# sleep3r/Diffusion-Handwriting-Generation.pytorch

Hardware: AMD Instinct MI355X
Metric: stroke-points/sec reverse-sampled (T=60, L=488) (higher is better)
Workload: dtype bf16; 1 GPU; configs[1]: batch=64 prompts/GPU, T=60, L=488, Lt=30, d_model=128/192/256, num_layers=2, diffusion_mode=new, random-init weights; global_batch=64, seq_len=488, parallelism=batch-shard x1 (no collectives)

## Files before the change

### diffusion-handwriting-generation.pytorch_amd/csrc/convblock.hip

```cpp
#include <algorithm>
#include <cstdlib>
#include "convblock_core.h"

namespace {

template <typename T, int BM, int CO, int NW, int OCC = 1, int UPC = 0, int CH = 0, int CIN = 0, int TIGHT = 0, int PP = 0>
__global__ __launch_bounds__(NW * 64) __attribute__((amdgpu_waves_per_eu(OCC * NW / 4, (OCC * NW / 4) < 2 ? 2 : OCC * NW / 4)))
void convblock_kernel(const ConvBlockParams p, const EncChain nx) {
  extern __shared__ __attribute__((aligned(16))) char smem[];
  constexpr int BMO = TIGHT == 2 ? BM : BM - 2 - 2 * TIGHT;
  const int tiles = (p.L + BMO - 1) / BMO;
  const int bid = xcd_swizzle(blockIdx.x, gridDim.x);
  convblock_body<T, BM, CO, NW, OCC, UPC, CH, CIN, TIGHT, PP>(p, nx, bid / tiles, (bid % tiles) * BMO, smem);
}

template <typename T, int BM, int CO, int NW, int OCC = 1, int UPC = 0, int CH = 0, int CIN = 0, int TIGHT = 0, int PP = 0>
hipError_t launch_t(const ConvBlockParams& p, hipStream_t st, const EncChain* nx = nullptr) {
  size_t lds = lds_bytes<T, BM, CO>(p.Cin, UPC ? p.up_cin : 0, TIGHT == 2 ? BM + 16 : BM);
  if (CH) lds = std::max(lds, (size_t)2 * BM * tile_stride<T>(CO) + 2 * 8 * BM * sizeof(float) + enc_a_text_kv_bytes<T, CO, BM>() + enc_a_param_bytes<T, CO>());
  if (lds > 160 * 1024 || (UPC && (p.Cin != UPC || p.up_cin % 32)) || (CH != 0) != (nx != nullptr)) return hipErrorInvalidValue;
  if (CIN && (p.Cin != CIN || (UPC && p.up_cin != up_skip_width<UPC>()))) return hipErrorInvalidValue;
  constexpr int BMO = TIGHT == 2 ? BM : BM - 2 - 2 * TIGHT;
  const int tiles = (p.L + BMO - 1) / BMO;
  hipLaunchKernelGGL((convblock_kernel<T, BM, CO, NW, OCC, UPC, CH, CIN, TIGHT, PP>), dim3(p.B * tiles), dim3(NW * 64), lds, st, p, nx ? *nx : EncChain{});
  return hipGetLastError();
}

template <typename T, int BM, int CO, int NW, int OCC = 1, int UPC = 0, int CH = 0, int CIN = 0, int TIGHT = 0, int PP = 0>
hipError_t attr() {
  return hipFuncSetAttribute(reinterpret_cast<const void*>(convblock_kernel<T, BM, CO, NW, OCC, UPC, CH, CIN, TIGHT, PP>),
                             hipFuncAttributeMaxDynamicSharedMemorySize, 160 * 1024);
}

constexpr int enc_cin(int CO) { return CO == 256 ? 192 : 128; }

}

hipError_t convblock_init() {
  hipError_t e;
#define A(...) if ((e = attr<__VA_ARGS__>()) != hipSuccess) return e
  A(bf16_t, 64, 128, 8); A(bf16_t, 128, 128, 8); A(bf16_t, 64, 128, 8, 2, 0, 0, 128); A(bf16_t, 64, 192, 8, 2, 0, 0, 128); A(bf16_t, 64, 192, 8);
  A(bf16_t, 64, 256, 8); A(bf16_t, 32, 256, 8); A(bf16_t, 48, 256, 8);
  A(bf16_t, 64, 128, 8, 1, 0, 0, 128); A(bf16_t, 128, 128, 8, 1, 0, 0, 128); A(bf16_t, 64, 192, 8, 1, 0, 0, 128);
  A(bf16_t, 64, 256, 8, 1, 0, 0, 192); A(bf16_t, 48, 256, 8, 1, 0, 0, 192);
  A(bf16_t, 64, 128, 8, 1, 192, 0, 192); A(bf16_t, 128, 128, 8, 1, 192, 0, 192); A(bf16_t, 64, 192, 8, 1, 256, 0, 256);
  A(bf16_t, 64, 256, 8, 1, 384, 0, 384); A(bf16_t, 48, 256, 8, 1, 384, 0, 384);
  A(bf16_t, 128, 128, 8, 1, 192, 0, 192, 1); A(bf16_t, 48, 256, 8, 1, 384, 0, 384, 1);
  A(bf16_t, 128, 128, 8, 1, 0, 0, 128, 0, 1); A(bf16_t, 128, 128, 8, 1, 192, 0, 192, 1, 1); A(bf16_t, 128, 128, 8, 1, 192, 0, 192, 0, 1);
  A(bf16_t, 32, 256, 8, 1, 0, 0, 192, 2); A(bf16_t, 32, 256, 8, 1, 384, 0, 384, 2);
  A(bf16_t, 64, 192, 8, 1, 0, 1, 128); A(bf16_t, 48, 256, 8, 1, 0, 1, 192); A(bf16_t, 64, 256, 8, 1, 0, 1, 192);
  A(bf16_t, 32, 256, 8, 1, 0, 1, 192, 2);
  A(float, 32, 128, 4); A(float, 32, 192, 4); A(float, 32, 256, 4);
#undef A
  return hipSuccess;
}

static long conv_wgs() {
  const char* e = getenv("DHW_CONV_WGS");
  return e ? atol(e) : 256;
}

static bool use_bm48(const ConvBlockParams& p) {
  if (const char* e = getenv("DHW_CONV_BM")) return atoi(e) == 48;
  const long t64 = (long)p.B * ((p.L + 61) / 62), t48 = (long)p.B * ((p.L + 45) / 46);
  return t64 < conv_wgs() && t48 <= conv_wgs() && t48 > t64;
}

static bool use_asym32(const ConvBlockParams& p) {
  static const bool on = !(getenv("DHW_CONV_ASYM") && atoi(getenv("DHW_CONV_ASYM")) == 0);
  if (!on || getenv("DHW_CONV_BM")) return false;
  const long t32 = (long)p.B * ((p.L + 31) / 32), t46 = (long)p.B * ((p.L + 45) / 46);
  return t32 <= conv_wgs() && t32 > t46;
}

static int conv_pp() {
  const char* e = getenv("DHW_CONV_PP");
  return e ? atoi(e) : 0;
}

hipError_t launch_convblock(int prec, const ConvBlockParams& p_in, hipStream_t st) {
  ConvBlockParams p = p_in;
  if (const char* e = getenv("DHW_CONV_STAGGER")) p.stagger = atoi(e);
  if (p.Cin % 32 || (p.L & 1) || (p.pool && p.out_f32) || (p.fuse_heads && !p.out_f32) || (!p.out && !p.fuse_heads)) return hipErrorInvalidValue;
  static const bool rt = getenv("DHW_CONV_RT") && atoi(getenv("DHW_CONV_RT"));
  if (p.up_h) {
    if (prec != PREC_BF16 || p.strokes || !p.up_w || !p.up_b || !p.up_low) return hipErrorInvalidValue;
    static const bool tight_ok = !(getenv("DHW_CONV_TIGHT") && atoi(getenv("DHW_CONV_TIGHT")) == 0);
    auto tight = [&](int bm) { return tight_ok && (p.L + bm - 5) / (bm - 4) == (p.L + bm - 3) / (bm - 2); };
    if (p.Cout == 128 && p.Cin == 192 && p.up_cin == 128) {
      const bool big = (long)p.B * ((p.L + 61) / 62) > conv_wgs() && lds_bytes<bf16_t, 128, 128>(p.Cin, p.up_cin) <= 160 * 1024;
      if (big && (conv_pp() & 2)) return tight(128) ? launch_t<bf16_t, 128, 128, 8, 1, 192, 0, 192, 1, 1>(p, st) : launch_t<bf16_t, 128, 128, 8, 1, 192, 0, 192, 0, 1>(p, st);
      if (big && tight(128)) return launch_t<bf16_t, 128, 128, 8, 1, 192, 0, 192, 1>(p, st);
      return big ? launch_t<bf16_t, 128, 128, 8, 1, 192, 0, 192>(p, st) : launch_t<bf16_t, 64, 128, 8, 1, 192, 0, 192>(p, st);
    }
    if (p.Cout == 192 && p.Cin == 256 && p.up_cin == 192) return launch_t<bf16_t, 64, 192, 8, 1, 256, 0, 256>(p, st);
    if (p.Cout == 256 && p.Cin == 384 && p.up_cin == 256) {
      if (use_asym32(p)) return launch_t<bf16_t, 32, 256, 8, 1, 384, 0, 384, 2>(p, st);
      if (use_bm48(p) && tight(48)) return launch_t<bf16_t, 48, 256, 8, 1, 384, 0, 384, 1>(p, st);
      return use_bm48(p) ? launch_t<bf16_t, 48, 256, 8, 1, 384, 0, 384>(p, st) : launch_t<bf16_t, 64, 256, 8, 1, 384, 0, 384>(p, st);
    }
    return hipErrorInvalidValue;
  }
  if (prec == PREC_BF16) {
    const bool sk = !rt && p.Cin == enc_cin(p.Cout);
    switch (p.Cout) {
      case 128: {
        const bool big = (long)p.B * ((p.L + 61) / 62) > conv_wgs() && lds_bytes<bf16_t, 128, 128>(p.Cin) <= 160 * 1024 &&
                         !(getenv("DHW_CONV_BM") && atoi(getenv("DHW_CONV_BM")) == 64);
        if (getenv("DHW_CONV_OCC") && atoi(getenv("DHW_CONV_OCC")) == 2 && sk && lds_bytes<bf16_t, 64, 128>(p.Cin) <= 80 * 1024)
          return launch_t<bf16_t, 64, 128, 8, 2, 0, 0, 128>(p, st);
        if (sk && big && (conv_pp() & 1)) return launch_t<bf16_t, 128, 128, 8, 1, 0, 0, 128, 0, 1>(p, st);
        if (sk) return big ? launch_t<bf16_t, 128, 128, 8, 1, 0, 0, 128>(p, st) : launch_t<bf16_t, 64, 128, 8, 1, 0, 0, 128>(p, st);
        return big ? launch_t<bf16_t, 128, 128, 8>(p, st) : launch_t<bf16_t, 64, 128, 8>(p, st);
      }
      case 192:
        if (getenv("DHW_CONV_OCC") && atoi(getenv("DHW_CONV_OCC")) == 2 && sk && lds_bytes<bf16_t, 64, 192>(p.Cin) <= 80 * 1024)
          return launch_t<bf16_t, 64, 192, 8, 2, 0, 0, 128>(p, st);
        return sk ? launch_t<bf16_t, 64, 192, 8, 1, 0, 0, 128>(p, st) : launch_t<bf16_t, 64, 192, 8>(p, st);
      case 256:
        if (sk && use_asym32(p)) return launch_t<bf16_t, 32, 256, 8, 1, 0, 0, 192, 2>(p, st);
        if (use_bm48(p)) return sk ? launch_t<bf16_t, 48, 256, 8, 1, 0, 0, 192>(p, st) : launch_t<bf16_t, 48, 256, 8>(p, st);
        if (getenv("DHW_CONV_BM") && atoi(getenv("DHW_CONV_BM")) == 32) return launch_t<bf16_t, 32, 256, 8>(p, st);
        return sk ? launch_t<bf16_t, 64, 256, 8, 1, 0, 0, 192>(p, st) : launch_t<bf16_t, 64, 256, 8>(p, st);
    }
  } else {
    switch (p.Cout) {
      case 128: return launch_t<float, 32, 128, 4>(p, st);
      case 192: return launch_t<float, 32, 192, 4>(p, st);
      case 256: return launch_t<float, 32, 256, 4>(p, st);
    }
  }
  return hipErrorInvalidValue;
}

bool convblock_chain_supported(int prec, const ConvBlockParams& p, const EncChain& chain) {
  if (prec != PREC_BF16 || chain.mode != 1 || chain.a.x || p.up_h || p.strokes || p.out_f32 || p.fuse_heads) return false;
  if (chain.a.d != p.Cout || chain.a.Lk != p.L || chain.a.B != p.B || (p.L & 1)) return false;
  if (getenv("DHW_CONV_BM") || getenv("DHW_CONV_OCC")) return false;
  return (p.Cout == 192 || p.Cout == 256) && p.Cin == enc_cin(p.Cout) && enclayer_supported(prec, chain.a.d, chain.a.heads);
}

bool convblock_chain_auto(const ConvBlockParams& p) { return p.Cout == 256 && use_asym32(p); }

hipError_t launch_convblock_chain(int prec, const ConvBlockParams& p, const EncChain& chain, hipStream_t st) {
  if (!convblock_chain_supported(prec, p, chain) || p.Cin % 32 || (!p.out)) return hipErrorInvalidValue;
  if (p.Cout == 192) return launch_t<bf16_t, 64, 192, 8, 1, 0, 1, 128>(p, st, &chain);
  if (use_asym32(p)) return launch_t<bf16_t, 32, 256, 8, 1, 0, 1, 192, 2>(p, st, &chain);
  return use_bm48(p) ? launch_t<bf16_t, 48, 256, 8, 1, 0, 1, 192>(p, st, &chain) : launch_t<bf16_t, 64, 256, 8, 1, 0, 1, 192>(p, st, &chain);
}
```

### diffusion-handwriting-generation.pytorch_amd/csrc/convblock_core.h

```cpp
#pragma once
#include <algorithm>
#include "enc_a_core.h"
#include "heads_core.h"

namespace {

#define CB_SILU(x) ((DHW_ABL & 8) ? (x) : silu_t<T>(x))
#define CB_SILU_TILES(NT_, MT_, v) do { if constexpr (!(DHW_ABL & 8)) silu_tiles2<T, NT_, MT_>(v); } while (0)
#define CB_BARRIER() do { if constexpr (!(DHW_ABL & 64)) lds_barrier(); } while (0)

#define STAMP(slot) DHW_STAMP_IF(p.stamps && (int)blockIdx.x == p.stagger && (threadIdx.x & 63) == 0, (threadIdx.x >> 6) * 16 + slot, __builtin_amdgcn_s_memrealtime())

template <typename T, int BM> __host__ __device__ constexpr int h2_stride(int CO) { return BM >= 128 ? CO * (int)sizeof(T) + 16 : tile_stride<T>(CO); }

template <int NT>
struct Epi {
  f32x4 bias[NT], gam[NT], bet[NT];
  DHW_DEV void load(const float* b, const float* g, const float* be, int n0) {
#pragma unroll
    for (int i = 0; i < NT; ++i) {
      bias[i] = *reinterpret_cast<const f32x4*>(b + n0 + 16 * i);
      gam[i] = *reinterpret_cast<const f32x4*>(g + n0 + 16 * i);
      bet[i] = *reinterpret_cast<const f32x4*>(be + n0 + 16 * i);
    }
  }
  DHW_DEV void load_bias(const float* b, int n0) {
#pragma unroll
    for (int i = 0; i < NT; ++i) {
      bias[i] = *reinterpret_cast<const f32x4*>(b + n0 + 16 * i);
      gam[i] = (f32x4){1, 1, 1, 1};
      bet[i] = (f32x4){0, 0, 0, 0};
    }
  }
};

template <int UPC> constexpr int up_skip_width() { return UPC == 384 ? 256 : UPC == 256 ? 192 : UPC == 192 ? 128 : 0; }
template <typename T, int BM, int CO, int NW, int OCC = 1, int UPC = 0, int CH = 0, int CIN = 0, int TIGHT = 0, int PP = 0, typename P, typename X>
DHW_DEV void convblock_body(const P& p, const X& nx, const int b, const int m0, char* smem) {
  constexpr int ES = sizeof(T), NTHR = NW * 64;
  constexpr bool SK = CIN != 0;
  constexpr int KT1 = 3 * CIN / 32;
  static_assert(UPC == 0 || CIN == 0 || CIN == UPC, "a fused input stage produces the block's own input width");
  constexpr bool ASYM = TIGHT == 2;
  constexpr int BMO = ASYM ? BM : BM - 2 - 2 * TIGHT;
  constexpr int RX = BMO + 4;
  constexpr int BM1 = ASYM ? BM + 16 : BM;
  constexpr int C1 = CO / 2;
  constexpr int T1 = C1 / 16, T2 = CO / 16;
  constexpr int WN1 = NW == 8 ? (T1 >= 8 ? 8 : (T1 == 6 ? 6 : 4)) : 2;
  constexpr int WM1 = NW == 8 ? (T1 >= 6 ? 1 : 2) : 2;
  constexpr bool TALL = NW == 8 && BM >= 128 && T2 == 8;
  constexpr int WN2 = NW == 8 ? (TALL ? 4 : (T2 % 8 == 0 ? 8 : 6)) : 4;
  constexpr int WM2 = TALL ? 2 : 1;
  constexpr int MT1 = BM1 / WM1 / 16, NT1 = T1 / WN1;
  constexpr int MT2 = BM / WM2 / 16, NT2 = T2 / WN2;
  static_assert(NT1 * WN1 == T1 && NT2 * WN2 == T2 && MT1 * 16 * WM1 == BM1 && WM1 * WN1 <= NW && WM2 * WN2 <= NW, "unsupported tile / wave layout");
  static_assert(!ASYM || WM1 == 1, "the asymmetric tiling: blocks with one row group in conv1");
  constexpr bool PPX = PP != 0;
  static_assert(!PPX || (TALL && WM1 == 2 && WN1 == 4 && CH == 0 && !ASYM && OCC == 1), "ping-pong: the 2 x 4 wave layouts of the tall tiles");
  constexpr int RING = (ES == 2 ? 24 : 12) * (CO == 256 ? 2 : 3) / 3 / (OCC * NW > 8 ? OCC : 1);

  const int Ls = sample_len(p.lens, p.lsh, b, p.L);
  if constexpr (DHW_LENS) { if (m0 >= Ls) return; }
  const int tid = body_tid(), lane = tid & 63, wave = __builtin_amdgcn_readfirstlane(tid >> 6);
  const int l15 = lane & 15, g = lane >> 4;
  const int Cin = SK ? CIN : p.Cin;
  const bool pp_lead = PPX && __builtin_amdgcn_readfirstlane(wave) >= NW / 2;
#define PP_BARRIER() do { if constexpr (PPX) CB_BARRIER(); } while (0)

  const int SX = tile_stride<T>(Cin), SH1 = tile_stride<T>(C1), SH2 = h2_stride<T, BM>(CO);
  char* XS = smem;
  char* XR = XS + RX * SX;
  char* H1 = XR + RX * SX;
  char* H2 = H1 + (BM1 + 2) * SH1;
  const float* gam = p.film + (size_t)b * p.film_bs;
  const float* bet = gam + p.film_tot;

  const bool act1 = WM1 * WN1 == NW || wave < WM1 * WN1, act2 = WM2 * WN2 == NW || wave < WM2 * WN2;
  const int wm1 = act1 ? wave / WN1 : 0, wn1 = act1 ? wave % WN1 : 0, row01 = wm1 * (BM1 / WM1), nt01 = wn1 * NT1;
  const int wm2 = act2 ? wave / WN2 : 0, wn2 = act2 ? wave % WN2 : 0, row02 = wm2 * (BM / WM2), nt02 = wn2 * NT2;
  const int n1 = nt01 * 16 + 4 * g, n2 = nt02 * 16 + 4 * g;
  const int KCin = Cin / 32;

  if constexpr (OCC == 2) {
    if (p.stagger && blockIdx.x >= gridDim.x / 2)
      for (int i = 0; i < p.stagger; ++i) __builtin_amdgcn_s_sleep(16);
  }
  STAMP(0);
  WRing<T, NT1, RING> ring1;
  Epi<NT1> ep1;
  auto fill1 = [&]() {
    const T* w = reinterpret_cast<const T*>(p.w_c1) + ((size_t)nt01 * KCin * 3 * 64 + lane) * 8;
    if constexpr (SK) ring1.template fill_s<KT1>(w);
    else ring1.fill(w, KCin * 3);
  };

  if constexpr (UPC != 0) {
    constexpr int RXP = (RX + 15) / 16 * 16, RH = RXP + 2, MTU = RXP / 16;
    constexpr int TU = UPC / 16, WNU = TU % 8 == 0 ? 8 : 4, WMU = NW / WNU, NTU = TU / WNU;
    constexpr int MTG = (MTU + WMU - 1) / WMU;
    static_assert(NTU * WNU == TU && NW == 8, "unsupported input width");
    const int wmu = wave / WNU, wnu = wave % WNU;
    const int ntu0 = wnu * NTU, nu = ntu0 * 16 + 4 * g, rowu0 = wmu * MTG * 16;
    constexpr int UCH = up_skip_width<UPC>();
    const int Ch = SK ? UCH : p.up_cin, KCh = Ch / 32, SHh = tile_stride<T>(Ch);
    char* HS = H1;
    WRing<T, NTU, (NTU * MTG >= 24 ? 12 : RING)> ringu;
    Epi<NTU> epu;
    {
      constexpr int CPRH = UCH * ES / 16, CPX = UPC * ES / 16;
      constexpr int UH = (RH * CPRH + NTHR - 1) / NTHR, UL = (RX * CPX + NTHR - 1) / NTHR;
      static_assert(SK, "the fused input stage is compiled for static widths");
      const char* src = reinterpret_cast<const char*>(p.up_h);
      const char* low = reinterpret_cast<const char*>(p.up_low);
      CopyRegs<UH> ch;
      CopyRegs<UL> cl;
      ch.load(RH * CPRH, tid, NTHR, [&](int id) { const int r = id / CPRH, cc = id - r * CPRH, lrow = min(max(m0 - 3 + r, 0), p.L - 1);
                                                  return reinterpret_cast<const uint4*>(src + ((size_t)(b * p.L + lrow) * UCH) * ES + (size_t)cc * 16); });
      cl.load(RX * CPX, tid, NTHR, [&](int id) { const int r = id / CPX, cc = id - r * CPX, lrow = min(max(m0 - 2 + r, 0), p.L - 1);
                                                 return reinterpret_cast<const uint4*>(low + ((size_t)(b * (p.L / 2) + (lrow >> 1)) * UPC) * ES + (size_t)cc * 16); });
      ch.store(RH * CPRH, tid, NTHR, [&](int id) { const int r = id / CPRH, cc = id - r * CPRH; return reinterpret_cast<uint4*>(HS + r * SHh + cc * 16); },
               [&](int id) { const int lrow = m0 - 3 + id / CPRH; return lrow >= 0 && lrow < Ls; });
      cl.store(RX * CPX, tid, NTHR, [&](int id) { const int r = id / CPX, cc = id - r * CPX; return reinterpret_cast<uint4*>(XR + r * SX + cc * 16); },
               [&](int id) { const int lrow = m0 - 2 + id / CPX; return lrow >= 0 && lrow < Ls; });
    }
    ringu.template fill_s<3 * UCH / 32>(reinterpret_cast<const T*>(p.up_w) + ((size_t)ntu0 * KCh * 3 * 64 + lane) * 8);
    epu.load_bias(p.up_b, nu);
    CB_BARRIER();
    STAMP(10);
    f32x4 acc[NTU][MTG];
    acc_zero(acc);
    ringu.template run_s<MTG, 3 * UCH / 32>(acc, HS + (rowu0 + l15) * SHh + g * 8 * ES, SHh, KCh);
    STAMP(11);
    if (act1) {
      fill1();
      ep1.load(p.b_c1, gam + p.f1, bet + p.f1, n1);
    }
    {
      auto keep = [&](int j) { const int lrow = m0 - 2 + rowu0 + j * 16 + l15; return lrow >= 0 && lrow < Ls; };
      auto valid = [&](int j) { return rowu0 + j * 16 + l15 < RX; };
#pragma unroll
      for (int i = 0; i < NTU; ++i)
#pragma unroll
        for (int j = 0; j < MTG; ++j) {
          const int r = min(rowu0 + j * 16 + l15, RX - 1);
          acc[i][j] = round_to<T>(acc[i][j] + epu.bias[i] + load4(reinterpret_cast<const T*>(XR + r * SX) + nu + 16 * i));
        }
      store_tiles<T, NTU, MTG>(lane, XR, SX, rowu0, nu, acc, keep, valid);
      CB_SILU_TILES(NTU, MTG, acc);
      store_tiles<T, NTU, MTG>(lane, XS, SX, rowu0, nu, acc, keep, valid);
    }
    STAMP(12);
  } else if (p.strokes && SK && NTHR % (CIN / 4 > 0 ? CIN / 4 : 1) == 0) {
    constexpr int CPR = CIN / 4 > 0 ? CIN / 4 : 1, IT = (RX * CPR + NTHR - 1) / NTHR, RSTEP = NTHR / CPR;
    const int c = (tid % CPR) * 4, r0 = tid / CPR;
    const f32x4 wa = *reinterpret_cast<const f32x4*>(p.in_w + c * 2), wb = *reinterpret_cast<const f32x4*>(p.in_w + c * 2 + 4);
    const f32x4 bb = *reinterpret_cast<const f32x4*>(p.in_b + c);
    float2 sp[IT];
#pragma unroll
    for (int it = 0; it < IT; ++it) {
      const int lrow = min(max(m0 - 2 + r0 + it * RSTEP, 0), p.L - 1);
      sp[it] = *reinterpret_cast<const float2*>(p.strokes + (size_t)(b * p.L + lrow) * 2);
    }
    const float w0[4] = {wa[0], wa[2], wb[0], wb[2]}, w1[4] = {wa[1], wa[3], wb[1], wb[3]};
#pragma unroll
    for (int it = 0; it < IT; ++it) {
      const int r = r0 + it * RSTEP, lrow = m0 - 2 + r;
      if (r < RX) {
        const bool in = lrow >= 0 && lrow < Ls;
        const float s0 = sp[it].x, s1 = sp[it].y;
        f32x4 v, sv;
#pragma unroll
        for (int k = 0; k < 4; ++k) {
          const float t = to_f(from_f<T>(w0[k] * s0 + w1[k] * s1 + bb[k]));
          v[k] = in ? t : 0.f;
          sv[k] = in ? CB_SILU(t) : 0.f;
        }
        store4(reinterpret_cast<T*>(XR + r * SX) + c, v);
        store4(reinterpret_cast<T*>(XS + r * SX) + c, sv);
      }
    }
  } else if (p.strokes) {
    const int cpr = Cin / 4;
    for (int id = tid; id < RX * cpr; id += NTHR) {
      const int r = id / cpr, c = (id - r * cpr) * 4;
      const int lrow = m0 - 2 + r;
      f32x4 v = (f32x4){0, 0, 0, 0}, sv = v;
      if (lrow >= 0 && lrow < Ls) {
        const float s0 = p.strokes[(size_t)(b * p.L + lrow) * 2], s1 = p.strokes[(size_t)(b * p.L + lrow) * 2 + 1];
#pragma unroll
        for (int k = 0; k < 4; ++k) {
          v[k] = to_f(from_f<T>(p.in_w[(c + k) * 2] * s0 + p.in_w[(c + k) * 2 + 1] * s1 + p.in_b[c + k]));
          sv[k] = CB_SILU(v[k]);
        }
      }
      store4(reinterpret_cast<T*>(XR + r * SX) + c, v);
      store4(reinterpret_cast<T*>(XS + r * SX) + c, sv);
    }
  } else {
    const int cpr = Cin * ES / 16;
    const int total = RX * cpr;
    const char* src = reinterpret_cast<const char*>(p.x);
    constexpr int U = 4;
    for (int base = tid; base < total; base += NTHR * U) {
      uint4 v[U];
#pragma unroll
      for (int u = 0; u < U; ++u) {
        const int id = min(base + u * NTHR, total - 1);
        const int r = id / cpr, cc = id - r * cpr;
        const int lrow = min(max(m0 - 2 + r, 0), p.L - 1);
        if constexpr (DHW_ABL & 32) v[u] = make_uint4(0, 0, 0, 0);
        else v[u] = *reinterpret_cast<const uint4*>(src + ((size_t)(b * p.L + lrow) * Cin) * ES + (size_t)cc * 16);
      }
#pragma unroll
      for (int u = 0; u < U; ++u) {
        const int id = base + u * NTHR;
        if (id < total) {
          const int r = id / cpr, cc = id - r * cpr;
          const int lrow = m0 - 2 + r;
          const bool k = lrow >= 0 && lrow < Ls;
          uint4 w = make_uint4(k ? v[u].x : 0u, k ? v[u].y : 0u, k ? v[u].z : 0u, k ? v[u].w : 0u);
          *reinterpret_cast<uint4*>(XR + r * SX + cc * 16) = w;
          *reinterpret_cast<uint4*>(XS + r * SX + cc * 16) = (DHW_ABL & 8) ? w : silu_piece<T>(w);
        }
      }
    }
  }
  if (UPC == 0 && act1) {
    fill1();
    ep1.load(p.b_c1, gam + p.f1, bet + p.f1, n1);
  }
  STAMP(15);
  CB_BARRIER();
  if constexpr (PPX) {
    if (!pp_lead) {
      for (int id = tid; id < 2 * SH1 / 16; id += NTHR / 2)
        *reinterpret_cast<uint4*>(H1 + BM1 * SH1 + id * 16) = make_uint4(0, 0, 0, 0);
      CB_BARRIER();
    }
  }
  STAMP(1);

  WRing<T, NT2, RING> ring2;
  Epi<NT2> ep2;

  {
    f32x4 acc[NT1][MT1];
    acc_zero(acc);
    if (act1) {
      if constexpr (SK) ring1.template run_s<MT1, KT1>(acc, XS + (row01 + l15) * SX + g * 8 * ES, SX, KCin);
      else ring1.template run<MT1>(acc, XS + (row01 + l15) * SX + g * 8 * ES, SX, KCin);
    }
    STAMP(2);
    PP_BARRIER();
    constexpr int KT2 = (C1 / 32) * 3;
    const T* w2 = reinterpret_cast<const T*>(p.w_c2) + ((size_t)nt02 * KT2 * 64 + lane) * 8;
    if (act2) { ring2.template fill_begin<KT2>(w2); ep2.load(p.b_c2, gam + p.f2, bet + p.f2, n2); }
    constexpr int ST1 = epilogue_steps<NT1, MT1>(), CH2 = decltype(ring2)::template fill_chunks<KT2>(), PER1 = (CH2 + ST1 - 1) / ST1;
    if (act1) {
      epilogue_pairs<T, NT1, MT1, !(DHW_ABL & 8)>(lane, H1, SH1, row01, n1, acc,
          [&](int i, const f32x4& a) { return (a + ep1.bias[i]) * ep1.gam[i] + ep1.bet[i]; },
          [&](int j) { const int srow = m0 - 1 + row01 + j * 16 + l15; return srow >= 0 && srow < Ls; },
          [](int) { return true; },
          [&](int step) {
            if (act2) {
#pragma unroll
              for (int c = 0; c < PER1; ++c) ring2.template fill_chunk<KT2>(step * PER1 + c);
            }
          });
    } else if (act2) {
#pragma unroll
      for (int c = 0; c < CH2; ++c) ring2.template fill_chunk<KT2>(c);
    }
    if constexpr (!PPX)
    for (int id = tid; id < 2 * SH1 / 16; id += NTHR)
      *reinterpret_cast<uint4*>(H1 + BM1 * SH1 + id * 16) = make_uint4(0, 0, 0, 0);
  }
  STAMP(13);
  CB_BARRIER();
  STAMP(3);

  if (act2) {
    f32x4 acc[NT2][MT2];
    acc_zero(acc);
    ring2.template run_s<MT2, (C1 / 32) * 3>(acc, H1 + (row02 + l15) * SH1 + g * 8 * ES, SH1, C1 / 32);
    STAMP(4);
    PP_BARRIER();
    {
      constexpr int KTF = CO / 32;
      ring2.template fill_begin<KTF>(reinterpret_cast<const T*>(p.w_fc) + ((size_t)nt02 * KTF * 64 + lane) * 8);
      constexpr int ST2 = epilogue_steps<NT2, MT2>(), CHF = decltype(ring2)::template fill_chunks<KTF>(), PER2 = (CHF + ST2 - 1) / ST2;
      epilogue_pairs<T, NT2, MT2, !(DHW_ABL & 8)>(lane, H2, SH2, row02, n2, acc,
          [&](int i, const f32x4& a) { return (a + ep2.bias[i]) * ep2.gam[i] + ep2.bet[i]; },
          [](int) { return true; }, [](int) { return true; },
          [&](int step) {
#pragma unroll
            for (int c = 0; c < PER2; ++c) ring2.template fill_chunk<KTF>(step * PER2 + c);
          });
    }
    ep2.load(p.b_fc, gam + p.f3, bet + p.f3, n2);
  }
  STAMP(14);
  CB_BARRIER();
  STAMP(5);

  f32x4 acc[NT2][MT2];
  acc_zero(acc);
  if (act2) {
    const T* wsk = reinterpret_cast<const T*>(p.w_skip) + ((size_t)nt02 * KCin * 3 * 64 + lane) * 8;
    constexpr bool FCX = SK && CO / 32 <= decltype(ring2)::D && DHW_ABL == 0;
    if constexpr (FCX) ring2.template run_n<MT2, CO / 32, KT1>(acc, H2 + (row02 + l15) * SH2 + g * 8 * ES, SH2, CO / 32, wsk);
    else ring2.template run_s<MT2, CO / 32>(acc, H2 + (row02 + l15) * SH2 + g * 8 * ES, SH2, CO / 32);
    STAMP(6);
    if constexpr (FCX) {}
    else if constexpr (SK) ring2.template fill_s<KT1>(wsk);
    else ring2.fill(wsk, KCin * 3);
#pragma unroll
    for (int i = 0; i < NT2; ++i)
#pragma unroll
      for (int j = 0; j < MT2; ++j) acc[i][j] = (acc[i][j] + ep2.bias[i]) * ep2.gam[i] + ep2.bet[i];
    ep2.load_bias(p.b_skip, n2);
    if constexpr (SK) ring2.template run_s<MT2, KT1>(acc, XR + (row02 + l15 + 1) * SX + g * 8 * ES, SX, KCin);
    else ring2.template run<MT2>(acc, XR + (row02 + l15 + 1) * SX + g * 8 * ES, SX, KCin);
  }
  STAMP(7);
  CB_BARRIER();
  if constexpr (PPX) { if (pp_lead && p.out_f32) CB_BARRIER(); }
  STAMP(8);

  const int rows_valid = min(BMO, Ls - m0);
  if (p.out_f32) {
    constexpr int SO = CO * 4 + 16;
    if (act2) {
#pragma unroll
      for (int i = 0; i < NT2; ++i)
#pragma unroll
        for (int j = 0; j < MT2; ++j)
          store4(reinterpret_cast<float*>(smem + (row02 + j * 16 + l15) * SO) + n2 + 16 * i, acc[i][j] + ep2.bias[i]);
    }
    CB_BARRIER();
    if (p.out)
      tile_copy_out<float>(smem, SO, reinterpret_cast<float*>(p.out) + (size_t)(b * p.L + m0) * CO, CO, rows_valid, CO, tid, NTHR);
    if (p.fuse_heads) {
      const int r = tid >> 2, q = tid & 3;
      float a0 = 0.f, a1 = 0.f, a2 = 0.f;
      if (r < rows_valid) {
        const float* xr = reinterpret_cast<const float*>(smem + r * SO);
#pragma unroll
        for (int c = q * 4; c < CO; c += 16) {
          const f32x4 v = *reinterpret_cast<const f32x4*>(xr + c);
          const f32x4 w0 = *reinterpret_cast<const f32x4*>(p.hp.w_out + c);
          const f32x4 w1 = *reinterpret_cast<const f32x4*>(p.hp.w_out + CO + c);
          const f32x4 w2 = *reinterpret_cast<const f32x4*>(p.hp.w_pen + c);
#pragma unroll
          for (int k = 0; k < 4; ++k) { a0 += v[k] * w0[k]; a1 += v[k] * w1[k]; a2 += v[k] * w2[k]; }
        }
      }
#pragma unroll
      for (int o = 2; o; o >>= 1) {
        a0 += __shfl_xor(a0, o);
        a1 += __shfl_xor(a1, o);
        a2 += __shfl_xor(a2, o);
      }
      if (r < rows_valid && q == 0) heads_finish(p.hp, (long)b * p.L + m0 + r, a0, a1, a2);
    }
  } else {
    if (act2) {
#pragma unroll
      for (int i = 0; i < NT2; ++i)
#pragma unroll
        for (int j = 0; j < MT2; ++j) acc[i][j] += ep2.bias[i];
      store_tiles<T, NT2, MT2>(lane, smem, SH2, row02, n2, acc);
    }
    CB_BARRIER();
    if constexpr (PPX) { if (pp_lead) CB_BARRIER(); }
    if constexpr (!(DHW_ABL & 16))
    tile_copy_out<T>(smem, SH2, reinterpret_cast<T*>(p.out) + (size_t)(b * p.L + m0) * CO, CO, rows_valid, CO, tid, NTHR);
    if (p.pool && !(DHW_ABL & 16))
      tile_copy_out_pool<T>(smem, SH2, reinterpret_cast<T*>(p.pool) + ((size_t)b * (p.L / 2) + m0 / 2) * CO, CO, rows_valid, CO, tid, NTHR);
    if constexpr (CH == 1) {
      static_assert(NW == 8 && sizeof(T) == 2, "enc_a_body runs on 8 waves");
      EncALds m;
      m.XR = smem;
      m.QR = smem + BM * SH2;
      m.red = reinterpret_cast<float*>(m.QR + BM * SH2);
      m.KT = reinterpret_cast<char*>(m.red) + 2 * 8 * BM * sizeof(float);
      m.VT = m.KT + 32 * tile_stride<T>(CO);
      m.VS = smem;
      m.PL = reinterpret_cast<float*>(m.KT + enc_a_text_kv_bytes<T, CO, BM>());
      enc_a_body<T, CO, BM, (ASYM ? 16 : 4)>(nx.a, m, b, m0, rows_valid);
    }
  }
  STAMP(9);
}

template <typename T, int BM, int CO>
inline size_t lds_bytes(int Cin, int up_cin = 0, int bm1 = BM) {
  const int rx = bm1 > BM ? BM + 4 : BM + 2;
  const size_t xt = (size_t)2 * rx * tile_stride<T>(Cin);
  const size_t ops = xt + (size_t)(bm1 + 2) * tile_stride<T>(CO / 2) + (size_t)BM * h2_stride<T, BM>(CO);
  const size_t outf = (size_t)BM * (CO * 4 + 16);
  const int mtu = (rx + 15) / 16, wmu = (Cin / 16) % 8 == 0 ? 1 : 2, rows_read = wmu * ((mtu + wmu - 1) / wmu) * 16 + 2;
  const size_t up = up_cin ? xt + (size_t)rows_read * tile_stride<T>(up_cin) : 0;
  return std::max(ops, std::max(outf, up));
}

}
```

### diffusion-handwriting-generation.pytorch_amd/csrc/dhw_common.h

```cpp
#pragma once
#include <hip/hip_runtime.h>
#include <stdint.h>

typedef __bf16 bf16_t;
typedef __bf16 bf16x8 __attribute__((ext_vector_type(8)));
typedef __bf16 bf16x4 __attribute__((ext_vector_type(4)));
typedef float f32x4 __attribute__((ext_vector_type(4)));

#define DHW_DEV __device__ __forceinline__

#ifdef DHW_OPAQUE_TID
__device__ __forceinline__ int body_tid() { int t = threadIdx.x; asm volatile("" : "+v"(t)); return t; }
#else
__device__ __forceinline__ int body_tid() { return threadIdx.x; }
#endif

#ifdef DHW_STAMPS
#define DHW_STAMP_IF(cond, slot_expr, value) do { if (cond) p.stamps[slot_expr] = (value); } while (0)
#else
#define DHW_STAMP_IF(cond, slot_expr, value) do { } while (0)
#endif

template <typename T> struct Frag;
template <> struct Frag<bf16_t> { bf16x8 v; };
template <> struct Frag<float> { f32x4 lo, hi; };

DHW_DEV void mma32(f32x4& acc, const Frag<bf16_t>& a, const Frag<bf16_t>& b) {
  acc = __builtin_amdgcn_mfma_f32_16x16x32_bf16(a.v, b.v, acc, 0, 0, 0);
}
DHW_DEV void mma32(f32x4& acc, const Frag<float>& a, const Frag<float>& b) {
  acc = __builtin_amdgcn_mfma_f32_16x16x4f32(a.lo[0], b.lo[0], acc, 0, 0, 0);
  acc = __builtin_amdgcn_mfma_f32_16x16x4f32(a.lo[1], b.lo[1], acc, 0, 0, 0);
  acc = __builtin_amdgcn_mfma_f32_16x16x4f32(a.lo[2], b.lo[2], acc, 0, 0, 0);
  acc = __builtin_amdgcn_mfma_f32_16x16x4f32(a.lo[3], b.lo[3], acc, 0, 0, 0);
  acc = __builtin_amdgcn_mfma_f32_16x16x4f32(a.hi[0], b.hi[0], acc, 0, 0, 0);
  acc = __builtin_amdgcn_mfma_f32_16x16x4f32(a.hi[1], b.hi[1], acc, 0, 0, 0);
  acc = __builtin_amdgcn_mfma_f32_16x16x4f32(a.hi[2], b.hi[2], acc, 0, 0, 0);
  acc = __builtin_amdgcn_mfma_f32_16x16x4f32(a.hi[3], b.hi[3], acc, 0, 0, 0);
}

DHW_DEV Frag<bf16_t> frag_load(const bf16_t* p) {
  Frag<bf16_t> f;
  f.v = *reinterpret_cast<const bf16x8*>(p);
  return f;
}
DHW_DEV Frag<float> frag_load(const float* p) {
  Frag<float> f;
  f.lo = *reinterpret_cast<const f32x4*>(p);
  f.hi = *reinterpret_cast<const f32x4*>(p + 4);
  return f;
}
template <typename T> DHW_DEV Frag<T> frag_zero();
template <> DHW_DEV Frag<bf16_t> frag_zero<bf16_t>() {
  Frag<bf16_t> f;
  for (int i = 0; i < 8; ++i) f.v[i] = (bf16_t)0.0f;
  return f;
}
template <> DHW_DEV Frag<float> frag_zero<float>() {
  Frag<float> f;
  f.lo = (f32x4){0, 0, 0, 0};
  f.hi = (f32x4){0, 0, 0, 0};
  return f;
}
DHW_DEV void frag_from_f32(Frag<bf16_t>& f, const f32x4& a, const f32x4& b) {
  for (int i = 0; i < 4; ++i) { f.v[i] = (bf16_t)a[i]; f.v[4 + i] = (bf16_t)b[i]; }
}
DHW_DEV void frag_from_f32(Frag<float>& f, const f32x4& a, const f32x4& b) { f.lo = a; f.hi = b; }

DHW_DEV Frag<bf16_t> frag_load_halves(const bf16_t* p0, const bf16_t* p1) {
  Frag<bf16_t> f;
  const bf16x4 a = *reinterpret_cast<const bf16x4*>(p0), b = *reinterpret_cast<const bf16x4*>(p1);
  f.v = __builtin_shufflevector(a, b, 0, 1, 2, 3, 4, 5, 6, 7);
  return f;
}
DHW_DEV Frag<float> frag_load_halves(const float* p0, const float* p1) {
  Frag<float> f;
  f.lo = *reinterpret_cast<const f32x4*>(p0);
  f.hi = *reinterpret_cast<const f32x4*>(p1);
  return f;
}

DHW_DEV f32x4 load4(const bf16_t* p) {
  bf16x4 v = *reinterpret_cast<const bf16x4*>(p);
  return (f32x4){(float)v[0], (float)v[1], (float)v[2], (float)v[3]};
}
DHW_DEV f32x4 load4(const float* p) { return *reinterpret_cast<const f32x4*>(p); }
DHW_DEV void store4(bf16_t* p, const f32x4& v) {
  bf16x4 o;
  for (int i = 0; i < 4; ++i) o[i] = (bf16_t)v[i];
  *reinterpret_cast<bf16x4*>(p) = o;
}
DHW_DEV void store4(float* p, const f32x4& v) { *reinterpret_cast<f32x4*>(p) = v; }

#include "xcd_swizzle.h"

template <int U, typename SrcF, typename DstF>
DHW_DEV void staged_copy(int total, int tid, int nthreads, SrcF src, DstF dst) {
  for (int base = tid; base < total; base += nthreads * U) {
    uint4 v[U];
#pragma unroll
    for (int u = 0; u < U; ++u) {
      const int id = base + u * nthreads;
      v[u] = make_uint4(0, 0, 0, 0);
      if (id < total) {
        const uint4* sp = src(id);
        if (sp) v[u] = *sp;
      }
    }
#pragma unroll
    for (int u = 0; u < U; ++u) {
      const int id = base + u * nthreads;
      if (id < total) *dst(id) = v[u];
    }
  }
}

template <int U, typename SrcF, typename KeepF, typename DstF>
DHW_DEV void staged_copy_clamped(int total, int tid, int nthreads, SrcF src, KeepF keep, DstF dst) {
  for (int base = tid; base < total; base += nthreads * U) {
    uint4 v[U];
#pragma unroll
    for (int u = 0; u < U; ++u) {
      const int id = min(base + u * nthreads, total - 1);
      v[u] = *src(id);
    }
#pragma unroll
    for (int u = 0; u < U; ++u) {
      const int id = base + u * nthreads;
      if (id < total) *dst(id) = keep(id) ? v[u] : make_uint4(0, 0, 0, 0);
    }
  }
}

template <int U>
struct CopyRegs {
  uint4 v[U];
  template <typename SrcF>
  DHW_DEV void load(int total, int tid, int nthreads, SrcF src) {
#pragma unroll
    for (int u = 0; u < U; ++u) {
      const int id = tid + u * nthreads;
      v[u] = *src(id < total ? id : total - 1);
    }
  }
  template <typename SinkF, typename KeepF>
  DHW_DEV void store_to(int total, int tid, int nthreads, SinkF sink, KeepF keep) {
#pragma unroll
    for (int u = 0; u < U; ++u) {
      const int id = tid + u * nthreads;
      if (id < total) {
        const bool k = keep(id);
        sink(id, make_uint4(k ? v[u].x : 0u, k ? v[u].y : 0u, k ? v[u].z : 0u, k ? v[u].w : 0u));
      }
    }
  }
  template <typename DstF, typename KeepF>
  DHW_DEV void store(int total, int tid, int nthreads, DstF dst, KeepF keep) {
#pragma unroll
    for (int u = 0; u < U; ++u) {
      const int id = tid + u * nthreads;
      if (id < total) {
        const bool k = keep(id);
        *dst(id) = make_uint4(k ? v[u].x : 0u, k ? v[u].y : 0u, k ? v[u].z : 0u, k ? v[u].w : 0u);
      }
    }
  }
};

DHW_DEV float xg_sum(float v) {
  auto a = __builtin_amdgcn_permlane16_swap(__float_as_uint(v), __float_as_uint(v), false, false);
  v = __uint_as_float(a[0]) + __uint_as_float(a[1]);
  auto b = __builtin_amdgcn_permlane32_swap(__float_as_uint(v), __float_as_uint(v), false, false);
  return __uint_as_float(b[0]) + __uint_as_float(b[1]);
}
DHW_DEV float xg_max(float v) {
  auto a = __builtin_amdgcn_permlane16_swap(__float_as_uint(v), __float_as_uint(v), false, false);
  v = fmaxf(__uint_as_float(a[0]), __uint_as_float(a[1]));
  auto b = __builtin_amdgcn_permlane32_swap(__float_as_uint(v), __float_as_uint(v), false, false);
  return fmaxf(__uint_as_float(b[0]), __uint_as_float(b[1]));
}

DHW_DEV void lds_barrier() { asm volatile("s_waitcnt lgkmcnt(0)\n\ts_barrier" ::: "memory"); }

DHW_DEV float silu_f(float x) { return x / (1.0f + __expf(-x)); }
template <typename T> DHW_DEV float silu_t(float x);
template <> DHW_DEV float silu_t<bf16_t>(float x) { return x * __builtin_amdgcn_rcpf(1.0f + __expf(-x)); }
template <> DHW_DEV float silu_t<float>(float x) { return silu_f(x); }
DHW_DEV float to_f(bf16_t x) { return (float)x; }
DHW_DEV float to_f(float x) { return x; }
template <typename T> DHW_DEV T from_f(float x) { return (T)x; }
```

### diffusion-handwriting-generation.pytorch_amd/csrc/epilogue.h

```cpp
#pragma once
#include <type_traits>
#include "dhw_common.h"

template <typename T, int N>
DHW_DEV void silu_tiles(f32x4 (&v)[N]) {
  if constexpr (sizeof(T) == 4) {
#pragma unroll
    for (int n = 0; n < N; ++n)
#pragma unroll
      for (int k = 0; k < 4; ++k) v[n][k] = silu_f(v[n][k]);
  } else {
    f32x4 t[N];
#pragma unroll
    for (int n = 0; n < N; ++n) t[n] = v[n] * -1.4426950408889634f;
#pragma unroll
    for (int n = 0; n < N; ++n)
#pragma unroll
      for (int k = 0; k < 4; ++k) t[n][k] = __builtin_amdgcn_exp2f(t[n][k]);
#pragma unroll
    for (int n = 0; n < N; ++n) t[n] = t[n] + 1.0f;
#pragma unroll
    for (int n = 0; n < N; ++n)
#pragma unroll
      for (int k = 0; k < 4; ++k) t[n][k] = __builtin_amdgcn_rcpf(t[n][k]);
#pragma unroll
    for (int n = 0; n < N; ++n) v[n] = v[n] * t[n];
  }
}
template <typename T, int N, int BASE = 0>
DHW_DEV void silu_flat(f32x4* flat) {
  constexpr int G = N - BASE >= 8 ? 8 : N - BASE;
  if constexpr (G > 0) {
    f32x4 grp[G];
#pragma unroll
    for (int n = 0; n < G; ++n) grp[n] = flat[BASE + n];
    silu_tiles<T, G>(grp);
#pragma unroll
    for (int n = 0; n < G; ++n) flat[BASE + n] = grp[n];
    silu_flat<T, N, BASE + G>(flat);
  }
}
template <typename T, int NT, int MT>
DHW_DEV void silu_tiles2(f32x4 (&v)[NT][MT]) { silu_flat<T, NT * MT>(&v[0][0]); }

template <typename T>
DHW_DEV f32x4 round_to(const f32x4& v) {
  if constexpr (sizeof(T) == 4) return v;
  else {
    const bf16x4 o = __builtin_convertvector(v, bf16x4);
    return (f32x4){(float)o[0], (float)o[1], (float)o[2], (float)o[3]};
  }
}

DHW_DEV uint2 pack4_bf16(const f32x4& v) {
  const bf16x4 o = __builtin_convertvector(v, bf16x4);
  return __builtin_bit_cast(uint2, o);
}

DHW_DEV void store_pair(int lane, bf16_t* p0, bf16_t* p1, const f32x4& v0, const f32x4& v1, bool keep0 = true, bool keep1 = true,
                        bool do0 = true, bool do1 = true) {
  uint2 a = pack4_bf16(v0), b = pack4_bf16(v1);
  a.x = keep0 ? a.x : 0u; a.y = keep0 ? a.y : 0u;
  b.x = keep1 ? b.x : 0u; b.y = keep1 ? b.y : 0u;
  const auto lo = __builtin_amdgcn_permlane16_swap(a.x, b.x, false, false);
  const auto hi = __builtin_amdgcn_permlane16_swap(a.y, b.y, false, false);
  const bool odd = (lane >> 4) & 1;
  char* dst = odd ? reinterpret_cast<char*>(p1) - 8 : reinterpret_cast<char*>(p0);
  if (odd ? do1 : do0) *reinterpret_cast<uint4*>(dst) = make_uint4(lo[0], hi[0], lo[1], hi[1]);
}
DHW_DEV void store_pair(int lane, float* p0, float* p1, const f32x4& v0, const f32x4& v1, bool keep0 = true, bool keep1 = true,
                        bool do0 = true, bool do1 = true) {
  if (do0) store4(p0, keep0 ? v0 : (f32x4){0, 0, 0, 0});
  if (do1) store4(p1, keep1 ? v1 : (f32x4){0, 0, 0, 0});
}
template <typename T>
DHW_DEV void store_one(T* p, const f32x4& v, bool keep = true, bool doit = true) {
  if (doit) store4(p, keep ? v : (f32x4){0, 0, 0, 0});
}

template <typename T, int NT, int MT, typename KeepF, typename ValidF>
DHW_DEV void store_tiles(int lane, char* tile, int S, int row0, int n0, const f32x4 (&v)[NT][MT], KeepF keep, ValidF valid) {
  const int l15 = lane & 15;
  constexpr int N = NT * MT;
  auto ptr = [&](int t) { const int i = t / MT, j = t - i * MT; return reinterpret_cast<T*>(tile + (row0 + j * 16 + l15) * S) + n0 + 16 * i; };
#pragma unroll
  for (int t = 0; t + 1 < N; t += 2) {
    const int j0 = t % MT, j1 = (t + 1) % MT;
    store_pair(lane, ptr(t), ptr(t + 1), v[t / MT][j0], v[(t + 1) / MT][j1], keep(j0), keep(j1), valid(j0), valid(j1));
  }
  if constexpr (N & 1) store_one<T>(ptr(N - 1), v[NT - 1][MT - 1], keep(MT - 1), valid(MT - 1));
}
template <typename T, int NT, int MT>
DHW_DEV void enc_store_tiles(int lane, char* tile, int S, int row0, int n0, const f32x4 (&v)[NT][MT]) {
  const int l15 = lane & 15;
#pragma unroll
  for (int i = 0; i < NT; ++i)
#pragma unroll
    for (int j = 0; j < MT; ++j) store4(reinterpret_cast<T*>(tile + (row0 + j * 16 + l15) * S) + n0 + 16 * i, v[i][j]);
}
template <typename T, int NT, int MT>
DHW_DEV void store_tiles(int lane, char* tile, int S, int row0, int n0, const f32x4 (&v)[NT][MT]) {
  store_tiles<T, NT, MT>(lane, tile, S, row0, n0, v, [](int) { return true; }, [](int) { return true; });
}

template <typename T>
DHW_DEV uint4 silu_piece(const uint4& w) {
  if constexpr (sizeof(T) == 4) {
    uint4 o = w;
    float* e = reinterpret_cast<float*>(&o);
#pragma unroll
    for (int i = 0; i < 4; ++i) e[i] = silu_f(e[i]);
    return o;
  } else {
    f32x4 v[2];
    v[0] = (f32x4){__uint_as_float(w.x << 16), __uint_as_float(w.x & 0xffff0000u), __uint_as_float(w.y << 16), __uint_as_float(w.y & 0xffff0000u)};
    v[1] = (f32x4){__uint_as_float(w.z << 16), __uint_as_float(w.z & 0xffff0000u), __uint_as_float(w.w << 16), __uint_as_float(w.w & 0xffff0000u)};
    silu_tiles<T, 2>(v);
    const uint2 a = pack4_bf16(v[0]), b = pack4_bf16(v[1]);
    return make_uint4(a.x, a.y, b.x, b.y);
  }
}

template <typename T, int NT, int MT, bool SILU, typename AffF, typename KeepF, typename ValidF, typename BetweenF>
DHW_DEV void epilogue_pairs(int lane, char* tile, int S, int row0, int n0, const f32x4 (&acc)[NT][MT], AffF aff, KeepF keep, ValidF valid, BetweenF between) {
  const int l15 = lane & 15;
  constexpr int N = NT * MT;
  auto ptr = [&](int t) { const int i = t / MT, j = t - i * MT; return reinterpret_cast<T*>(tile + (row0 + j * 16 + l15) * S) + n0 + 16 * i; };
#pragma unroll
  for (int t = 0; t + 1 < N; t += 2) {
    const int i0 = t / MT, j0 = t % MT, i1 = (t + 1) / MT, j1 = (t + 1) % MT;
    f32x4 v[2] = {aff(i0, acc[i0][j0]), aff(i1, acc[i1][j1])};
    if constexpr (SILU) silu_tiles<T, 2>(v);
    store_pair(lane, ptr(t), ptr(t + 1), v[0], v[1], keep(j0), keep(j1), valid(j0), valid(j1));
    between(t / 2);
    __builtin_amdgcn_sched_barrier(0);
  }
  if constexpr (N & 1) {
    f32x4 v[1] = {aff(NT - 1, acc[NT - 1][MT - 1])};
    if constexpr (SILU) silu_tiles<T, 1>(v);
    store_one<T>(ptr(N - 1), v[0], keep(MT - 1), valid(MT - 1));
    between(N / 2);
    __builtin_amdgcn_sched_barrier(0);
  }
}
template <int NT, int MT> constexpr int epilogue_steps() { return (NT * MT + 1) / 2; }
```

### diffusion-handwriting-generation.pytorch_amd/csrc/gemm_core.h

```cpp
#pragma once
#include "dhw_common.h"
#include "epilogue.h"

template <typename T> constexpr int OPAD = sizeof(T) == 2 ? 32 : 16;
template <typename T> __host__ __device__ constexpr int tile_stride(int C) { return C * (int)sizeof(T) + OPAD<T>; }

DHW_DEV void keep_alive(const Frag<bf16_t>& f) { asm volatile("" ::"v"(f.v)); }
DHW_DEV void keep_alive(const Frag<float>& f) { asm volatile("" ::"v"(f.lo), "v"(f.hi)); }

#ifndef DHW_ABL
#define DHW_ABL 0
#endif
template <typename T, int NT, int RING = (sizeof(T) == 2 ? 24 : 12), int DMAX = 8>
struct WRing {
  static constexpr int D0 = RING / NT;
  static constexpr int D = D0 < 2 ? 2 : (D0 > DMAX ? DMAX : D0);
  Frag<T> q[D][NT];
  const T* base;
  int KT, KTS;

  DHW_DEV void fill(const T* __restrict__ wbase, int kt, int kts = 0) {
    base = wbase;
    KT = kt;
    KTS = kts ? kts : kt;
#pragma unroll
    for (int d = 0; d < D; ++d) {
      const int k = d < KT ? d : KT - 1;
#pragma unroll
      for (int i = 0; i < NT; ++i) q[d][i] = frag_load(base + ((size_t)i * KTS + k) * 512);
    }
  }

  template <int MT, int ABL = DHW_ABL>
  DHW_DEV void run(f32x4 (&acc)[NT][MT], const char* abase, int stride, int KC) {
    constexpr int ES = sizeof(T);
    int aoff = 0, kc = 0;
    const int tap_step = stride - (KC - 1) * 32 * ES;
    auto step = [&](int d, int knext) {
      Frag<T> a[MT];
#pragma unroll
      for (int j = 0; j < MT; ++j) {
        if constexpr (ABL & 4) a[j] = frag_zero<T>();
        else a[j] = frag_load(reinterpret_cast<const T*>(abase + j * 16 * stride + aoff));
      }
#pragma unroll
      for (int i = 0; i < NT; ++i)
#pragma unroll
        for (int j = 0; j < MT; ++j) {
          if constexpr (ABL & 1) { keep_alive(q[d][i]); keep_alive(a[j]); }
          else mma32(acc[i][j], q[d][i], a[j]);
        }
      const int kn = knext < KT ? knext : KT - 1;
      if constexpr (!(ABL & 2)) {
#pragma unroll
        for (int i = 0; i < NT; ++i) q[d][i] = frag_load(base + ((size_t)i * KTS + kn) * 512);
      }
      const bool wrap = ++kc == KC;
      aoff += wrap ? tap_step : 32 * ES;
      kc = wrap ? 0 : kc;
    };
    int kt = 0;
    for (; kt + D <= KT; kt += D) {
#pragma unroll
      for (int d = 0; d < D; ++d) step(d, kt + d + D);
    }
#pragma unroll
    for (int d = 0; d < D; ++d)
      if (kt + d < KT) step(d, KT - 1);
  }

  DHW_DEV void load_chunk(int d, int k) {
#pragma unroll
    for (int i = 0; i < NT; ++i) q[d][i] = frag_load(base + ((size_t)i * KTS + k) * 512);
  }
  template <int KT_>
  DHW_DEV void fill_begin(const T* __restrict__ wbase, int kts = 0) {
    base = wbase;
    KT = KT_;
    KTS = kts ? kts : KT_;
  }
  template <int KT_>
  static constexpr int fill_chunks() { return D < KT_ ? D : KT_; }
  template <int KT_>
  DHW_DEV void fill_chunk(int d) {
    if (d < fill_chunks<KT_>()) load_chunk(d, d);
  }
  template <int KT_, int A, int B>
  DHW_DEV void fill_range() {
#pragma unroll
    for (int d = A; d < B; ++d) fill_chunk<KT_>(d);
  }
  template <int KT_>
  DHW_DEV void fill_s(const T* __restrict__ wbase, int kts = 0) {
    base = wbase;
    KT = KT_;
    KTS = kts ? kts : KT_;
#pragma unroll
    for (int d = 0; d < (D < KT_ ? D : KT_); ++d) {
      load_chunk(d, d);
    }
  }
  template <int MT> static constexpr int act_ahead() { return MT == 1 ? 3 : 1; }
  template <int MT, int KT_, int PF>
  DHW_DEV void run_p(f32x4 (&acc)[NT][MT], const char* abase, int stride, int KC) {
    constexpr int ES = sizeof(T), NB = PF + 1;
    static_assert(D % NB == 0, "the rolled part of the loop needs static fragment-ring indices");
    constexpr int NR = KT_ > D ? KT_ - D : 0, G = NR / D;
    Frag<T> a[NB][MT];
    int aoff = 0, kc = 0;
    const int tap_step = stride - (KC - 1) * 32 * ES;
    auto request = [&](int slot) {
#pragma unroll
      for (int j = 0; j < MT; ++j) a[slot][j] = frag_load(reinterpret_cast<const T*>(abase + j * 16 * stride + aoff));
      const bool wrap = ++kc == KC;
      aoff += wrap ? tap_step : 32 * ES;
      kc = wrap ? 0 : kc;
    };
    auto step = [&](int d, int slot, bool more, bool reload, int knext) {
      if (more) request((slot + PF) % NB);
      __builtin_amdgcn_sched_barrier(0);
#pragma unroll
      for (int i = 0; i < NT; ++i)
#pragma unroll
        for (int j = 0; j < MT; ++j) mma32(acc[i][j], q[d][i], a[slot][j]);
      if (reload) load_chunk(d, knext);
      __builtin_amdgcn_sched_barrier(0);
    };
#pragma unroll
    for (int c = 0; c < PF; ++c)
      if (c < KT_) request(c);
    int kt = 0;
#pragma unroll 1
    for (int g = 0; g < G; ++g, kt += D) {
#pragma unroll
      for (int d = 0; d < D; ++d) step(d, d % NB, true, true, kt + d + D);
    }
#pragma unroll
    for (int j = 0; j < KT_ - G * D; ++j) step(j % D, (G * D + j) % NB, G * D + j + PF < KT_, G * D + j + D < KT_, G * D + j + D);
  }
  template <int MT, int KT_, int ABL = DHW_ABL>
  DHW_DEV void run_s(f32x4 (&acc)[NT][MT], const char* abase, int stride, int KC) {
    constexpr int PF = act_ahead<MT>();
    if constexpr (ABL == 0 && D % (PF + 1) == 0 && PF < D) {
      run_p<MT, KT_, PF>(acc, abase, stride, KC);
      return;
    }
    constexpr int ES = sizeof(T);
    constexpr int NR = KT_ > D ? KT_ - D : 0;
    constexpr int G = NR / D;
    int aoff = 0, kc = 0;
    const int tap_step = stride - (KC - 1) * 32 * ES;
    auto step = [&](int d, bool reload, int knext) {
      Frag<T> a[MT];
#pragma unroll
      for (int j = 0; j < MT; ++j) {
        if constexpr (ABL & 4) a[j] = frag_zero<T>();
        else a[j] = frag_load(reinterpret_cast<const T*>(abase + j * 16 * stride + aoff));
      }
#pragma unroll
      for (int i = 0; i < NT; ++i)
#pragma unroll
        for (int j = 0; j < MT; ++j) {
          if constexpr (ABL & 1) { keep_alive(q[d][i]); keep_alive(a[j]); }
          else mma32(acc[i][j], q[d][i], a[j]);
        }
      if constexpr (!(ABL & 2)) {
        if (reload) load_chunk(d, knext);
      }
      const bool wrap = ++kc == KC;
      aoff += wrap ? tap_step : 32 * ES;
      kc = wrap ? 0 : kc;
    };
    int kt = 0;
#pragma unroll 1
    for (int g = 0; g < G; ++g, kt += D) {
#pragma unroll
      for (int d = 0; d < D; ++d) step(d, true, kt + d + D);
    }
#pragma unroll
    for (int j = 0; j < KT_ - G * D; ++j) step(j % D, G * D + j + D < KT_, G * D + j + D);
  }

  template <int KT_> static constexpr int eff_depth() { return D < KT_ ? D : KT_; }

  template <int MT, int KT_, int KTN_>
  DHW_DEV void run_n(f32x4 (&acc)[NT][MT], const char* abase, int stride, int KC, const T* __restrict__ nbase, int nkts = 0) {
    static_assert(KT_ <= D, "run_n: the stage must fit the ring");
    constexpr int ES = sizeof(T), DN = eff_depth<KTN_>();
    constexpr int XTRA = DN > KT_ ? DN - KT_ : 0, PER = (XTRA + KT_ - 1) / KT_;
    const int nKTS = nkts ? nkts : KTN_;
    int aoff = 0, kc = 0;
    const int tap_step = stride - (KC - 1) * 32 * ES;
    constexpr int PF = act_ahead<MT>(), NB = PF + 1;
    Frag<T> a[NB][MT];
    auto request = [&](int slot) {
#pragma unroll
      for (int j = 0; j < MT; ++j) a[slot][j] = frag_load(reinterpret_cast<const T*>(abase + j * 16 * stride + aoff));
      const bool wrap = ++kc == KC;
      aoff += wrap ? tap_step : 32 * ES;
      kc = wrap ? 0 : kc;
    };
    auto next_chunk = [&](int c) {
#pragma unroll
      for (int i = 0; i < NT; ++i) q[c][i] = frag_load(nbase + ((size_t)i * nKTS + c) * 512);
    };
#pragma unroll
    for (int c = 0; c < PF; ++c)
      if (c < KT_) request(c);
#pragma unroll
    for (int s = 0; s < KT_; ++s) {
      if (s + PF < KT_) request((s + PF) % NB);
      __builtin_amdgcn_sched_barrier(0);
#pragma unroll
      for (int i = 0; i < NT; ++i)
#pragma unroll
        for (int j = 0; j < MT; ++j) mma32(acc[i][j], q[s][i], a[s % NB][j]);
      if (s < DN) next_chunk(s);
#pragma unroll
      for (int e = 0; e < PER; ++e)
        if (KT_ + s * PER + e < DN) next_chunk(KT_ + s * PER + e);
      __builtin_amdgcn_sched_barrier(0);
    }
    base = nbase; KT = KTN_; KTS = nKTS;
  }
};

template <typename T, int MT, int NT, int RING = (sizeof(T) == 2 ? 24 : 12), int ABL = 0>
DHW_DEV void mainloop(f32x4 (&acc)[NT][MT], const T* __restrict__ wbase, const char* abase, int stride, int KC, int taps,
                      int KTS = 0) {
  WRing<T, NT, RING> ring;
  ring.fill(wbase, KC * taps, KTS);
  ring.template run<MT, ABL>(acc, abase, stride, KC);
}

template <typename T>
DHW_DEV void tile_copy_out(const char* lds, int S, T* gdst, int gs, int rows_valid, int C, int tid, int nthreads) {
  constexpr int ES = sizeof(T), EPV = 16 / ES;
  const int cpr = C / EPV;
  const int total = rows_valid * cpr;
  for (int id = tid; id < total; id += nthreads) {
    const int r = id / cpr, cc = id - r * cpr;
    *reinterpret_cast<uint4*>(gdst + (size_t)r * gs + cc * EPV) = *reinterpret_cast<const uint4*>(lds + r * S + cc * 16);
  }
}
template <typename T>
DHW_DEV void tile_copy_out_pool(const char* lds, int S, T* gdst, int gs, int rows_valid_in, int C, int tid, int nthreads) {
  constexpr int ES = sizeof(T), EPV = 16 / ES;
  const int cpr = C / EPV;
  const int total = (rows_valid_in / 2) * cpr;
  for (int id = tid; id < total; id += nthreads) {
    const int r = id / cpr, cc = id - r * cpr;
    uint4 a = *reinterpret_cast<const uint4*>(lds + (2 * r) * S + cc * 16);
    const uint4 b = *reinterpret_cast<const uint4*>(lds + (2 * r + 1) * S + cc * 16);
    T* ea = reinterpret_cast<T*>(&a);
    const T* eb = reinterpret_cast<const T*>(&b);
#pragma unroll
    for (int k = 0; k < EPV; ++k) ea[k] = from_f<T>(0.5f * (to_f(ea[k]) + to_f(eb[k])));
    *reinterpret_cast<uint4*>(gdst + (size_t)r * gs + cc * EPV) = a;
  }
}

template <int NT, int MT>
DHW_DEV void acc_zero(f32x4 (&acc)[NT][MT]) {
#pragma unroll
  for (int i = 0; i < NT; ++i)
#pragma unroll
    for (int j = 0; j < MT; ++j) acc[i][j] = (f32x4){0, 0, 0, 0};
}

template <int MT, int NT, int WN, int ROWS>
DHW_DEV void layernorm_rows(f32x4 (&acc)[NT][MT], float* red, int wn, int row0, int lane, int N, bool act = true) {
  const int l15 = lane & 15, g = lane >> 4;
  float mean[MT], rstd[MT];
#pragma unroll
  for (int j = 0; j < MT; ++j) {
    float s = 0.f;
#pragma unroll
    for (int i = 0; i < NT; ++i) s += acc[i][j][0] + acc[i][j][1] + acc[i][j][2] + acc[i][j][3];
    s = xg_sum(s);
    if (g == 0 && act) red[wn * ROWS + row0 + j * 16 + l15] = s;
  }
  lds_barrier();
  const float invn = 1.0f / (float)N;
#pragma unroll
  for (int j = 0; j < MT; ++j) {
    float s = 0.f;
#pragma unroll
    for (int w = 0; w < WN; ++w) s += red[w * ROWS + row0 + j * 16 + l15];
    mean[j] = s * invn;
  }
#pragma unroll
  for (int j = 0; j < MT; ++j) {
    float s = 0.f;
#pragma unroll
    for (int i = 0; i < NT; ++i)
#pragma unroll
      for (int r = 0; r < 4; ++r) { const float d = acc[i][j][r] - mean[j]; s += d * d; }
    s = xg_sum(s);
    if (g == 0 && act) red[(WN + wn) * ROWS + row0 + j * 16 + l15] = s;
  }
  lds_barrier();
#pragma unroll
  for (int j = 0; j < MT; ++j) {
    float s = 0.f;
#pragma unroll
    for (int w = 0; w < WN; ++w) s += red[(WN + w) * ROWS + row0 + j * 16 + l15];
    rstd[j] = rsqrtf(s * invn + 1e-6f);
  }
#pragma unroll
  for (int i = 0; i < NT; ++i)
#pragma unroll
    for (int j = 0; j < MT; ++j) acc[i][j] = (acc[i][j] - mean[j]) * rstd[j];
}

struct NoHook { DHW_DEV void operator()() const {} };
template <int MT, int NT, int WN, int ROWS, typename Mid = NoHook>
DHW_DEV void layernorm_rows_1pass(f32x4 (&acc)[NT][MT], float* red, int wn, int row0, int lane, int N, bool act = true, Mid mid = Mid()) {
  const int l15 = lane & 15, g = lane >> 4;
#pragma unroll
  for (int j = 0; j < MT; ++j) {
    float s = 0.f, q = 0.f;
#pragma unroll
    for (int i = 0; i < NT; ++i)
#pragma unroll
      for (int r = 0; r < 4; ++r) { s += acc[i][j][r]; q += acc[i][j][r] * acc[i][j][r]; }
    s = xg_sum(s); q = xg_sum(q);
    if (g == 0 && act) {
      red[wn * ROWS + row0 + j * 16 + l15] = s;
      red[(WN + wn) * ROWS + row0 + j * 16 + l15] = q;
    }
  }
  mid();
  lds_barrier();
  const float invn = 1.0f / (float)N;
#pragma unroll
  for (int j = 0; j < MT; ++j) {
    float s = 0.f, q = 0.f;
#pragma unroll
    for (int w = 0; w < WN; ++w) { s += red[w * ROWS + row0 + j * 16 + l15]; q += red[(WN + w) * ROWS + row0 + j * 16 + l15]; }
    const float mean = s * invn;
    const float rstd = rsqrtf(fmaxf(q * invn - mean * mean, 0.f) + 1e-6f);
#pragma unroll
    for (int i = 0; i < NT; ++i) acc[i][j] = (acc[i][j] - mean) * rstd;
  }
}

template <typename T, int MT, int NT, int WN, int ROWS, typename Mid = NoHook>
DHW_DEV void ln_rows(f32x4 (&acc)[NT][MT], float* red, int wn, int row0, int lane, int N, bool act = true, Mid mid = Mid()) {
  if constexpr (sizeof(T) == 4) { mid(); layernorm_rows<MT, NT, WN, ROWS>(acc, red, wn, row0, lane, N, act); }
  else layernorm_rows_1pass<MT, NT, WN, ROWS, Mid>(acc, red, wn, row0, lane, N, act, mid);
}
```

Measured before the change: 1.783 million stroke-points/s.

## Use buffer loads with hardware bounds checks and scalar weight addressing in convblock

Activation and stroke loads now go through AMD buffer resources sized to the valid rows, so out-of-range rows read as zero in hardware. This replaces per-element clamping and masking arithmetic. Weight-fragment addressing is split into a scalar base plus a per-lane offset with immediate-offset grouping, and tile copy-out uses flat row-major indexing. The fp32 output path is compiled only for the configurations that use it, which should cut code size and register pressure elsewhere. The risk is that it depends on correct buffer range sizes and on the zero-fill semantics for halo rows.

```diff
diff --git a/diffusion-handwriting-generation.pytorch_amd/csrc/convblock.hip b/diffusion-handwriting-generation.pytorch_amd/csrc/convblock.hip
--- a/diffusion-handwriting-generation.pytorch_amd/csrc/convblock.hip
+++ b/diffusion-handwriting-generation.pytorch_amd/csrc/convblock.hip
@@ -20,6 +20,7 @@
   if (CH) lds = std::max(lds, (size_t)2 * BM * tile_stride<T>(CO) + 2 * 8 * BM * sizeof(float) + enc_a_text_kv_bytes<T, CO, BM>() + enc_a_param_bytes<T, CO>());
   if (lds > 160 * 1024 || (UPC && (p.Cin != UPC || p.up_cin % 32)) || (CH != 0) != (nx != nullptr)) return hipErrorInvalidValue;
   if (CIN && (p.Cin != CIN || (UPC && p.up_cin != up_skip_width<UPC>()))) return hipErrorInvalidValue;
+  if (p.out_f32 && !has_f32_out<T, CO, UPC, CH, CIN>()) return hipErrorInvalidValue;
   constexpr int BMO = TIGHT == 2 ? BM : BM - 2 - 2 * TIGHT;
   const int tiles = (p.L + BMO - 1) / BMO;
   hipLaunchKernelGGL((convblock_kernel<T, BM, CO, NW, OCC, UPC, CH, CIN, TIGHT, PP>), dim3(p.B * tiles), dim3(NW * 64), lds, st, p, nx ? *nx : EncChain{});
@@ -102,7 +103,7 @@
     return hipErrorInvalidValue;
   }
   if (prec == PREC_BF16) {
-    const bool sk = !rt && p.Cin == enc_cin(p.Cout);
+    const bool sk = !rt && p.Cin == enc_cin(p.Cout) && !p.out_f32;
     switch (p.Cout) {
       case 128: {
         const bool big = (long)p.B * ((p.L + 61) / 62) > conv_wgs() && lds_bytes<bf16_t, 128, 128>(p.Cin) <= 160 * 1024 &&
diff --git a/diffusion-handwriting-generation.pytorch_amd/csrc/convblock_core.h b/diffusion-handwriting-generation.pytorch_amd/csrc/convblock_core.h
--- a/diffusion-handwriting-generation.pytorch_amd/csrc/convblock_core.h
+++ b/diffusion-handwriting-generation.pytorch_amd/csrc/convblock_core.h
@@ -34,6 +34,7 @@
   }
 };
 
+template <typename T, int CO, int UPC, int CH, int CIN> constexpr bool has_f32_out() { return sizeof(T) == 4 || (CO == 128 && CH == 0 && (UPC != 0 || CIN == 0)); }
 template <int UPC> constexpr int up_skip_width() { return UPC == 384 ? 256 : UPC == 256 ? 192 : UPC == 192 ? 128 : 0; }
 template <typename T, int BM, int CO, int NW, int OCC = 1, int UPC = 0, int CH = 0, int CIN = 0, int TIGHT = 0, int PP = 0, typename P, typename X>
 DHW_DEV void convblock_body(const P& p, const X& nx, const int b, const int m0, char* smem) {
@@ -57,6 +58,7 @@
   static_assert(NT1 * WN1 == T1 && NT2 * WN2 == T2 && MT1 * 16 * WM1 == BM1 && WM1 * WN1 <= NW && WM2 * WN2 <= NW, "unsupported tile / wave layout");
   static_assert(!ASYM || WM1 == 1, "the asymmetric tiling: blocks with one row group in conv1");
   constexpr bool PPX = PP != 0;
+  constexpr bool F32O = has_f32_out<T, CO, UPC, CH, CIN>();
   static_assert(!PPX || (TALL && WM1 == 2 && WN1 == 4 && CH == 0 && !ASYM && OCC == 1), "ping-pong: the 2 x 4 wave layouts of the tall tiles");
   constexpr int RING = (ES == 2 ? 24 : 12) * (CO == 256 ? 2 : 3) / 3 / (OCC * NW > 8 ? OCC : 1);
 
@@ -65,6 +67,7 @@
   const int tid = body_tid(), lane = tid & 63, wave = __builtin_amdgcn_readfirstlane(tid >> 6);
   const int l15 = lane & 15, g = lane >> 4;
   const int Cin = SK ? CIN : p.Cin;
+  auto wsrc = [&](const void* w, int frag0) { return WSrc<T>{reinterpret_cast<const T*>(w) + (size_t)frag0 * 512, (uint32_t)(lane * 8 * ES)}; };
   const bool pp_lead = PPX && __builtin_amdgcn_readfirstlane(wave) >= NW / 2;
 #define PP_BARRIER() do { if constexpr (PPX) CB_BARRIER(); } while (0)
 
@@ -87,10 +90,10 @@
       for (int i = 0; i < p.stagger; ++i) __builtin_amdgcn_s_sleep(16);
   }
   STAMP(0);
-  WRing<T, NT1, RING> ring1;
+  WRing<T, NT1, RING, 8, true> ring1;
   Epi<NT1> ep1;
   auto fill1 = [&]() {
-    const T* w = reinterpret_cast<const T*>(p.w_c1) + ((size_t)nt01 * KCin * 3 * 64 + lane) * 8;
+    const WSrc<T> w = wsrc(p.w_c1, nt01 * KCin * 3);
     if constexpr (SK) ring1.template fill_s<KT1>(w);
     else ring1.fill(w, KCin * 3);
   };
@@ -105,26 +108,23 @@
     constexpr int UCH = up_skip_width<UPC>();
     const int Ch = SK ? UCH : p.up_cin, KCh = Ch / 32, SHh = tile_stride<T>(Ch);
     char* HS = H1;
-    WRing<T, NTU, (NTU * MTG >= 24 ? 12 : RING)> ringu;
+    WRing<T, NTU, (NTU * MTG >= 24 ? 12 : RING), 8, true> ringu;
     Epi<NTU> epu;
     {
       constexpr int CPRH = UCH * ES / 16, CPX = UPC * ES / 16;
       constexpr int UH = (RH * CPRH + NTHR - 1) / NTHR, UL = (RX * CPX + NTHR - 1) / NTHR;
       static_assert(SK, "the fused input stage is compiled for static widths");
-      const char* src = reinterpret_cast<const char*>(p.up_h);
-      const char* low = reinterpret_cast<const char*>(p.up_low);
+      constexpr int RBH = UCH * ES, RBX = UPC * ES;
+      const RowsBuf hb(reinterpret_cast<const char*>(p.up_h) + (size_t)b * p.L * RBH, Ls * RBH);
+      const RowsBuf lb(reinterpret_cast<const char*>(p.up_low) + (size_t)b * (p.L / 2) * RBX, (Ls / 2) * RBX);
       CopyRegs<UH> ch;
       CopyRegs<UL> cl;
-      ch.load(RH * CPRH, tid, NTHR, [&](int id) { const int r = id / CPRH, cc = id - r * CPRH, lrow = min(max(m0 - 3 + r, 0), p.L - 1);
-                                                  return reinterpret_cast<const uint4*>(src + ((size_t)(b * p.L + lrow) * UCH) * ES + (size_t)cc * 16); });
-      cl.load(RX * CPX, tid, NTHR, [&](int id) { const int r = id / CPX, cc = id - r * CPX, lrow = min(max(m0 - 2 + r, 0), p.L - 1);
-                                                 return reinterpret_cast<const uint4*>(low + ((size_t)(b * (p.L / 2) + (lrow >> 1)) * UPC) * ES + (size_t)cc * 16); });
-      ch.store(RH * CPRH, tid, NTHR, [&](int id) { const int r = id / CPRH, cc = id - r * CPRH; return reinterpret_cast<uint4*>(HS + r * SHh + cc * 16); },
-               [&](int id) { const int lrow = m0 - 3 + id / CPRH; return lrow >= 0 && lrow < Ls; });
-      cl.store(RX * CPX, tid, NTHR, [&](int id) { const int r = id / CPX, cc = id - r * CPX; return reinterpret_cast<uint4*>(XR + r * SX + cc * 16); },
-               [&](int id) { const int lrow = m0 - 2 + id / CPX; return lrow >= 0 && lrow < Ls; });
-    }
-    ringu.template fill_s<3 * UCH / 32>(reinterpret_cast<const T*>(p.up_w) + ((size_t)ntu0 * KCh * 3 * 64 + lane) * 8);
+      ch.load_with(tid, NTHR, [&](int id) { return hb.load16((m0 - 3) * RBH + id * 16); });
+      cl.load_with(tid, NTHR, [&](int id) { const int r = id / CPX, cc = id - r * CPX; return lb.load16(((m0 - 2) / 2 + (r >> 1)) * RBX + cc * 16); });
+      ch.store_all(RH * CPRH, tid, NTHR, [&](int id) { return reinterpret_cast<uint4*>(HS + id * 16 + (id / CPRH) * (SHh - RBH)); });
+      cl.store_all(RX * CPX, tid, NTHR, [&](int id) { return reinterpret_cast<uint4*>(XR + id * 16 + (id / CPX) * (SX - RBX)); });
+    }
+    ringu.template fill_s<3 * UCH / 32>(wsrc(p.up_w, ntu0 * KCh * 3));
     epu.load_bias(p.up_b, nu);
     CB_BARRIER();
     STAMP(10);
@@ -137,8 +137,8 @@
       ep1.load(p.b_c1, gam + p.f1, bet + p.f1, n1);
     }
     {
-      auto keep = [&](int j) { const int lrow = m0 - 2 + rowu0 + j * 16 + l15; return lrow >= 0 && lrow < Ls; };
-      auto valid = [&](int j) { return rowu0 + j * 16 + l15 < RX; };
+      auto keep = [&](int j) { return tile_row_in(m0 - 2 + rowu0, j, l15, Ls); };
+      auto valid = [&](int j) { return l15 < RX - rowu0 - j * 16; };
 #pragma unroll
       for (int i = 0; i < NTU; ++i)
 #pragma unroll
@@ -157,17 +157,15 @@
     const f32x4 wa = *reinterpret_cast<const f32x4*>(p.in_w + c * 2), wb = *reinterpret_cast<const f32x4*>(p.in_w + c * 2 + 4);
     const f32x4 bb = *reinterpret_cast<const f32x4*>(p.in_b + c);
     float2 sp[IT];
-#pragma unroll
-    for (int it = 0; it < IT; ++it) {
-      const int lrow = min(max(m0 - 2 + r0 + it * RSTEP, 0), p.L - 1);
-      sp[it] = *reinterpret_cast<const float2*>(p.strokes + (size_t)(b * p.L + lrow) * 2);
-    }
+    const RowsBuf sb(p.strokes + (size_t)b * p.L * 2, Ls * 8);
+#pragma unroll
+    for (int it = 0; it < IT; ++it) sp[it] = sb.load_f2((m0 - 2 + r0 + it * RSTEP) * 8);
     const float w0[4] = {wa[0], wa[2], wb[0], wb[2]}, w1[4] = {wa[1], wa[3], wb[1], wb[3]};
 #pragma unroll
     for (int it = 0; it < IT; ++it) {
       const int r = r0 + it * RSTEP, lrow = m0 - 2 + r;
       if (r < RX) {
-        const bool in = lrow >= 0 && lrow < Ls;
+        const bool in = (unsigned)lrow < (unsigned)Ls;
         const float s0 = sp[it].x, s1 = sp[it].y;
         f32x4 v, sv;
 #pragma unroll
@@ -198,30 +196,25 @@
       store4(reinterpret_cast<T*>(XS + r * SX) + c, sv);
     }
   } else {
-    const int cpr = Cin * ES / 16;
+    const int RB = Cin * ES, cpr = RB / 16;
     const int total = RX * cpr;
-    const char* src = reinterpret_cast<const char*>(p.x);
+    const RowsBuf xb(reinterpret_cast<const char*>(p.x) + (size_t)b * p.L * RB, Ls * RB);
+    const int g0 = (m0 - 2) * RB;
     constexpr int U = 4;
     for (int base = tid; base < total; base += NTHR * U) {
       uint4 v[U];
 #pragma unroll
       for (int u = 0; u < U; ++u) {
-        const int id = min(base + u * NTHR, total - 1);
-        const int r = id / cpr, cc = id - r * cpr;
-        const int lrow = min(max(m0 - 2 + r, 0), p.L - 1);
         if constexpr (DHW_ABL & 32) v[u] = make_uint4(0, 0, 0, 0);
-        else v[u] = *reinterpret_cast<const uint4*>(src + ((size_t)(b * p.L + lrow) * Cin) * ES + (size_t)cc * 16);
+        else v[u] = xb.load16(g0 + (base + u * NTHR) * 16);
       }
 #pragma unroll
       for (int u = 0; u < U; ++u) {
         const int id = base + u * NTHR;
         if (id < total) {
-          const int r = id / cpr, cc = id - r * cpr;
-          const int lrow = m0 - 2 + r;
-          const bool k = lrow >= 0 && lrow < Ls;
-          uint4 w = make_uint4(k ? v[u].x : 0u, k ? v[u].y : 0u, k ? v[u].z : 0u, k ? v[u].w : 0u);
-          *reinterpret_cast<uint4*>(XR + r * SX + cc * 16) = w;
-          *reinterpret_cast<uint4*>(XS + r * SX + cc * 16) = (DHW_ABL & 8) ? w : silu_piece<T>(w);
+          const int o = id * 16 + (id / cpr) * (SX - RB);
+          *reinterpret_cast<uint4*>(XR + o) = v[u];
+          *reinterpret_cast<uint4*>(XS + o) = (DHW_ABL & 8) ? v[u] : silu_piece<T>(v[u]);
         }
       }
     }
@@ -241,7 +234,7 @@
   }
   STAMP(1);
 
-  WRing<T, NT2, RING> ring2;
+  WRing<T, NT2, RING, 8, true> ring2;
   Epi<NT2> ep2;
 
   {
@@ -254,13 +247,13 @@
     STAMP(2);
     PP_BARRIER();
     constexpr int KT2 = (C1 / 32) * 3;
-    const T* w2 = reinterpret_cast<const T*>(p.w_c2) + ((size_t)nt02 * KT2 * 64 + lane) * 8;
+    const WSrc<T> w2 = wsrc(p.w_c2, nt02 * KT2);
     if (act2) { ring2.template fill_begin<KT2>(w2); ep2.load(p.b_c2, gam + p.f2, bet + p.f2, n2); }
     constexpr int ST1 = epilogue_steps<NT1, MT1>(), CH2 = decltype(ring2)::template fill_chunks<KT2>(), PER1 = (CH2 + ST1 - 1) / ST1;
     if (act1) {
       epilogue_pairs<T, NT1, MT1, !(DHW_ABL & 8)>(lane, H1, SH1, row01, n1, acc,
           [&](int i, const f32x4& a) { return (a + ep1.bias[i]) * ep1.gam[i] + ep1.bet[i]; },
-          [&](int j) { const int srow = m0 - 1 + row01 + j * 16 + l15; return srow >= 0 && srow < Ls; },
+          [&](int j) { return tile_row_in(m0 - 1 + row01, j, l15, Ls); },
           [](int) { return true; },
           [&](int step) {
             if (act2) {
@@ -288,7 +281,7 @@
     PP_BARRIER();
     {
       constexpr int KTF = CO / 32;
-      ring2.template fill_begin<KTF>(reinterpret_cast<const T*>(p.w_fc) + ((size_t)nt02 * KTF * 64 + lane) * 8);
+      ring2.template fill_begin<KTF>(wsrc(p.w_fc, nt02 * KTF));
       constexpr int ST2 = epilogue_steps<NT2, MT2>(), CHF = decltype(ring2)::template fill_chunks<KTF>(), PER2 = (CHF + ST2 - 1) / ST2;
       epilogue_pairs<T, NT2, MT2, !(DHW_ABL & 8)>(lane, H2, SH2, row02, n2, acc,
           [&](int i, const f32x4& a) { return (a + ep2.bias[i]) * ep2.gam[i] + ep2.bet[i]; },
@@ -307,7 +300,7 @@
   f32x4 acc[NT2][MT2];
   acc_zero(acc);
   if (act2) {
-    const T* wsk = reinterpret_cast<const T*>(p.w_skip) + ((size_t)nt02 * KCin * 3 * 64 + lane) * 8;
+    const WSrc<T> wsk = wsrc(p.w_skip, nt02 * KCin * 3);
     constexpr bool FCX = SK && CO / 32 <= decltype(ring2)::D && DHW_ABL == 0;
     if constexpr (FCX) ring2.template run_n<MT2, CO / 32, KT1>(acc, H2 + (row02 + l15) * SH2 + g * 8 * ES, SH2, CO / 32, wsk);
     else ring2.template run_s<MT2, CO / 32>(acc, H2 + (row02 + l15) * SH2 + g * 8 * ES, SH2, CO / 32);
@@ -325,11 +318,11 @@
   }
   STAMP(7);
   CB_BARRIER();
-  if constexpr (PPX) { if (pp_lead && p.out_f32) CB_BARRIER(); }
+  if constexpr (PPX) { if (pp_lead && F32O && p.out_f32) CB_BARRIER(); }
   STAMP(8);
 
   const int rows_valid = min(BMO, Ls - m0);
-  if (p.out_f32) {
+  if (F32O && p.out_f32) {
     constexpr int SO = CO * 4 + 16;
     if (act2) {
 #pragma unroll
@@ -340,7 +333,7 @@
     }
     CB_BARRIER();
     if (p.out)
-      tile_copy_out<float>(smem, SO, reinterpret_cast<float*>(p.out) + (size_t)(b * p.L + m0) * CO, CO, rows_valid, CO, tid, NTHR);
+      tile_copy_out_rows<float, CO>(smem, SO, reinterpret_cast<float*>(p.out) + (size_t)(b * p.L + m0) * CO, rows_valid, tid, NTHR);
     if (p.fuse_heads) {
       const int r = tid >> 2, q = tid & 3;
       float a0 = 0.f, a1 = 0.f, a2 = 0.f;
@@ -375,9 +368,9 @@
     CB_BARRIER();
     if constexpr (PPX) { if (pp_lead) CB_BARRIER(); }
     if constexpr (!(DHW_ABL & 16))
-    tile_copy_out<T>(smem, SH2, reinterpret_cast<T*>(p.out) + (size_t)(b * p.L + m0) * CO, CO, rows_valid, CO, tid, NTHR);
+    tile_copy_out_rows<T, CO>(smem, SH2, reinterpret_cast<T*>(p.out) + (size_t)(b * p.L + m0) * CO, rows_valid, tid, NTHR);
     if (p.pool && !(DHW_ABL & 16))
-      tile_copy_out_pool<T>(smem, SH2, reinterpret_cast<T*>(p.pool) + ((size_t)b * (p.L / 2) + m0 / 2) * CO, CO, rows_valid, CO, tid, NTHR);
+      tile_copy_out_pool_rows<T, CO>(smem, SH2, reinterpret_cast<T*>(p.pool) + ((size_t)b * (p.L / 2) + m0 / 2) * CO, rows_valid, tid, NTHR);
     if constexpr (CH == 1) {
       static_assert(NW == 8 && sizeof(T) == 2, "enc_a_body runs on 8 waves");
       EncALds m;
diff --git a/diffusion-handwriting-generation.pytorch_amd/csrc/dhw_common.h b/diffusion-handwriting-generation.pytorch_amd/csrc/dhw_common.h
--- a/diffusion-handwriting-generation.pytorch_amd/csrc/dhw_common.h
+++ b/diffusion-handwriting-generation.pytorch_amd/csrc/dhw_common.h
@@ -94,6 +94,21 @@
 
 #include "xcd_swizzle.h"
 
+typedef unsigned int u32x4_t __attribute__((ext_vector_type(4)));
+typedef unsigned int u32x2_t __attribute__((ext_vector_type(2)));
+struct RowsBuf {
+  decltype(__builtin_amdgcn_make_buffer_rsrc((void*)nullptr, (short)0, 0, 0)) r;
+  DHW_DEV RowsBuf(const void* base, int bytes) : r(__builtin_amdgcn_make_buffer_rsrc(const_cast<void*>(base), (short)0, bytes, 0x00020000)) {}
+  DHW_DEV uint4 load16(int off) const {
+    const u32x4_t v = __builtin_amdgcn_raw_buffer_load_b128(r, off, 0, 0);
+    return make_uint4(v[0], v[1], v[2], v[3]);
+  }
+  DHW_DEV float2 load_f2(int off) const {
+    const u32x2_t v = __builtin_amdgcn_raw_buffer_load_b64(r, off, 0, 0);
+    return make_float2(__uint_as_float(v[0]), __uint_as_float(v[1]));
+  }
+};
+
 template <int U, typename SrcF, typename DstF>
 DHW_DEV void staged_copy(int total, int tid, int nthreads, SrcF src, DstF dst) {
   for (int base = tid; base < total; base += nthreads * U) {
@@ -141,6 +156,19 @@
     for (int u = 0; u < U; ++u) {
       const int id = tid + u * nthreads;
       v[u] = *src(id < total ? id : total - 1);
+    }
+  }
+  template <typename LoadF>
+  DHW_DEV void load_with(int tid, int nthreads, LoadF ld) {
+#pragma unroll
+    for (int u = 0; u < U; ++u) v[u] = ld(tid + u * nthreads);
+  }
+  template <typename DstF>
+  DHW_DEV void store_all(int total, int tid, int nthreads, DstF dst) {
+#pragma unroll
+    for (int u = 0; u < U; ++u) {
+      const int id = tid + u * nthreads;
+      if (id < total) *dst(id) = v[u];
     }
   }
   template <typename SinkF, typename KeepF>
diff --git a/diffusion-handwriting-generation.pytorch_amd/csrc/epilogue.h b/diffusion-handwriting-generation.pytorch_amd/csrc/epilogue.h
--- a/diffusion-handwriting-generation.pytorch_amd/csrc/epilogue.h
+++ b/diffusion-handwriting-generation.pytorch_amd/csrc/epilogue.h
@@ -68,6 +68,14 @@
   char* dst = odd ? reinterpret_cast<char*>(p1) - 8 : reinterpret_cast<char*>(p0);
   if (odd ? do1 : do0) *reinterpret_cast<uint4*>(dst) = make_uint4(lo[0], hi[0], lo[1], hi[1]);
 }
+DHW_DEV void store_pair_at(char* dst, const f32x4& v0, const f32x4& v1, bool keep0, bool keep1, bool wr) {
+  uint2 a = pack4_bf16(v0), b = pack4_bf16(v1);
+  a.x = keep0 ? a.x : 0u; a.y = keep0 ? a.y : 0u;
+  b.x = keep1 ? b.x : 0u; b.y = keep1 ? b.y : 0u;
+  const auto lo = __builtin_amdgcn_permlane16_swap(a.x, b.x, false, false);
+  const auto hi = __builtin_amdgcn_permlane16_swap(a.y, b.y, false, false);
+  if (wr) *reinterpret_cast<uint4*>(dst) = make_uint4(lo[0], hi[0], lo[1], hi[1]);
+}
 DHW_DEV void store_pair(int lane, float* p0, float* p1, const f32x4& v0, const f32x4& v1, bool keep0 = true, bool keep1 = true,
                         bool do0 = true, bool do1 = true) {
   if (do0) store4(p0, keep0 ? v0 : (f32x4){0, 0, 0, 0});
@@ -78,15 +86,37 @@
   if (doit) store4(p, keep ? v : (f32x4){0, 0, 0, 0});
 }
 
+template <typename T, int MT>
+struct PairDst {
+  char* same;
+  char* wrap;
+  bool odd;
+  DHW_DEV PairDst(int lane, char* tile, int S, int row0, int n0) {
+    constexpr int ES = sizeof(T);
+    odd = (lane >> 4) & 1;
+    char* const pb = tile + (row0 + (lane & 15)) * S + n0 * ES;
+    same = pb + (odd ? 16 * S - 8 : 0);
+    wrap = pb + (odd ? 16 * ES - (MT - 1) * 16 * S - 8 : 0);
+  }
+  DHW_DEV char* at(int t, int S) const {
+    const int i = t / MT, j = t - i * MT;
+    return (j + 1 < MT ? same : wrap) + j * 16 * S + i * 16 * (int)sizeof(T);
+  }
+};
+
+DHW_DEV bool tile_row_in(int s0, int j, int l15, int n) { return j == 0 ? (unsigned)(s0 + l15) < (unsigned)n : l15 < n - s0 - 16 * j; }
+
 template <typename T, int NT, int MT, typename KeepF, typename ValidF>
 DHW_DEV void store_tiles(int lane, char* tile, int S, int row0, int n0, const f32x4 (&v)[NT][MT], KeepF keep, ValidF valid) {
   const int l15 = lane & 15;
   constexpr int N = NT * MT;
   auto ptr = [&](int t) { const int i = t / MT, j = t - i * MT; return reinterpret_cast<T*>(tile + (row0 + j * 16 + l15) * S) + n0 + 16 * i; };
+  const PairDst<T, MT> pd(lane, tile, S, row0, n0);
 #pragma unroll
   for (int t = 0; t + 1 < N; t += 2) {
     const int j0 = t % MT, j1 = (t + 1) % MT;
-    store_pair(lane, ptr(t), ptr(t + 1), v[t / MT][j0], v[(t + 1) / MT][j1], keep(j0), keep(j1), valid(j0), valid(j1));
+    if constexpr (sizeof(T) == 2) store_pair_at(pd.at(t, S), v[t / MT][j0], v[(t + 1) / MT][j1], keep(j0), keep(j1), pd.odd ? valid(j1) : valid(j0));
+    else store_pair(lane, ptr(t), ptr(t + 1), v[t / MT][j0], v[(t + 1) / MT][j1], keep(j0), keep(j1), valid(j0), valid(j1));
   }
   if constexpr (N & 1) store_one<T>(ptr(N - 1), v[NT - 1][MT - 1], keep(MT - 1), valid(MT - 1));
 }
@@ -126,12 +156,14 @@
   const int l15 = lane & 15;
   constexpr int N = NT * MT;
   auto ptr = [&](int t) { const int i = t / MT, j = t - i * MT; return reinterpret_cast<T*>(tile + (row0 + j * 16 + l15) * S) + n0 + 16 * i; };
+  const PairDst<T, MT> pd(lane, tile, S, row0, n0);
 #pragma unroll
   for (int t = 0; t + 1 < N; t += 2) {
     const int i0 = t / MT, j0 = t % MT, i1 = (t + 1) / MT, j1 = (t + 1) % MT;
     f32x4 v[2] = {aff(i0, acc[i0][j0]), aff(i1, acc[i1][j1])};
     if constexpr (SILU) silu_tiles<T, 2>(v);
-    store_pair(lane, ptr(t), ptr(t + 1), v[0], v[1], keep(j0), keep(j1), valid(j0), valid(j1));
+    if constexpr (sizeof(T) == 2) store_pair_at(pd.at(t, S), v[0], v[1], keep(j0), keep(j1), pd.odd ? valid(j1) : valid(j0));
+    else store_pair(lane, ptr(t), ptr(t + 1), v[0], v[1], keep(j0), keep(j1), valid(j0), valid(j1));
     between(t / 2);
     __builtin_amdgcn_sched_barrier(0);
   }
diff --git a/diffusion-handwriting-generation.pytorch_amd/csrc/gemm_core.h b/diffusion-handwriting-generation.pytorch_amd/csrc/gemm_core.h
--- a/diffusion-handwriting-generation.pytorch_amd/csrc/gemm_core.h
+++ b/diffusion-handwriting-generation.pytorch_amd/csrc/gemm_core.h
@@ -1,4 +1,5 @@
 #pragma once
+#include <type_traits>
 #include "dhw_common.h"
 #include "epilogue.h"
 
@@ -11,23 +12,42 @@
 #ifndef DHW_ABL
 #define DHW_ABL 0
 #endif
-template <typename T, int NT, int RING = (sizeof(T) == 2 ? 24 : 12), int DMAX = 8>
+template <typename T> struct WSrc { const T* base; uint32_t lane; };
+template <typename T, int NT, int RING = (sizeof(T) == 2 ? 24 : 12), int DMAX = 8, bool UB = false>
 struct WRing {
   static constexpr int D0 = RING / NT;
   static constexpr int D = D0 < 2 ? 2 : (D0 > DMAX ? DMAX : D0);
   Frag<T> q[D][NT];
+  using Src = std::conditional_t<UB, WSrc<T>, const T* __restrict__>;
+  static constexpr int FB = 512 * (int)sizeof(T), IMM = 4096 / FB;
   const T* base;
+  uint32_t loff;
   int KT, KTS;
-
-  DHW_DEV void fill(const T* __restrict__ wbase, int kt, int kts = 0) {
-    base = wbase;
+  DHW_DEV void src(const Src& w) {
+    if constexpr (UB) { base = w.base; loff = w.lane; }
+    else { base = w; loff = 0; }
+  }
+  DHW_DEV Frag<T> wfrag(int i, int kts, int kv, int kc) const { return wfrag_of(base, loff, i, kts, kv, kc); }
+  static DHW_DEV Frag<T> wfrag_of(const T* base, uint32_t loff, int i, int kts, int kv, int kc) {
+    if constexpr (UB) {
+      const int fc = i * kts + kc;
+      const char* b = reinterpret_cast<const char*>(base) + ((size_t)kv + (size_t)(fc / IMM * IMM)) * FB;
+      asm("" : "+s"(b));
+      return frag_load(reinterpret_cast<const T*>(b + (fc % IMM) * FB + loff));
+    } else {
+      const int k = kv + kc;
+      return frag_load(base + ((size_t)i * kts + k) * 512);
+    }
+  }
+  DHW_DEV void fill(Src wbase, int kt, int kts = 0) {
+    src(wbase);
     KT = kt;
     KTS = kts ? kts : kt;
 #pragma unroll
     for (int d = 0; d < D; ++d) {
       const int k = d < KT ? d : KT - 1;
 #pragma unroll
-      for (int i = 0; i < NT; ++i) q[d][i] = frag_load(base + ((size_t)i * KTS + k) * 512);
+      for (int i = 0; i < NT; ++i) q[d][i] = wfrag(i, KTS, k, 0);
     }
   }
 
@@ -53,7 +73,7 @@
       const int kn = knext < KT ? knext : KT - 1;
       if constexpr (!(ABL & 2)) {
 #pragma unroll
-        for (int i = 0; i < NT; ++i) q[d][i] = frag_load(base + ((size_t)i * KTS + kn) * 512);
+        for (int i = 0; i < NT; ++i) q[d][i] = wfrag(i, KTS, kn, 0);
       }
       const bool wrap = ++kc == KC;
       aoff += wrap ? tap_step : 32 * ES;
@@ -69,13 +89,13 @@
       if (kt + d < KT) step(d, KT - 1);
   }
 
-  DHW_DEV void load_chunk(int d, int k) {
-#pragma unroll
-    for (int i = 0; i < NT; ++i) q[d][i] = frag_load(base + ((size_t)i * KTS + k) * 512);
+  DHW_DEV void load_chunk(int d, int kv, int kc) {
+#pragma unroll
+    for (int i = 0; i < NT; ++i) q[d][i] = wfrag(i, KTS, kv, kc);
   }
   template <int KT_>
-  DHW_DEV void fill_begin(const T* __restrict__ wbase, int kts = 0) {
-    base = wbase;
+  DHW_DEV void fill_begin(Src wbase, int kts = 0) {
+    src(wbase);
     KT = KT_;
     KTS = kts ? kts : KT_;
   }
@@ -83,7 +103,7 @@
   static constexpr int fill_chunks() { return D < KT_ ? D : KT_; }
   template <int KT_>
   DHW_DEV void fill_chunk(int d) {
-    if (d < fill_chunks<KT_>()) load_chunk(d, d);
+    if (d < fill_chunks<KT_>()) load_chunk(d, 0, d);
   }
   template <int KT_, int A, int B>
   DHW_DEV void fill_range() {
@@ -91,13 +111,13 @@
     for (int d = A; d < B; ++d) fill_chunk<KT_>(d);
   }
   template <int KT_>
-  DHW_DEV void fill_s(const T* __restrict__ wbase, int kts = 0) {
-    base = wbase;
+  DHW_DEV void fill_s(Src wbase, int kts = 0) {
+    src(wbase);
     KT = KT_;
     KTS = kts ? kts : KT_;
 #pragma unroll
     for (int d = 0; d < (D < KT_ ? D : KT_); ++d) {
-      load_chunk(d, d);
+      load_chunk(d, 0, d);
     }
   }
   template <int MT> static constexpr int act_ahead() { return MT == 1 ? 3 : 1; }
@@ -116,14 +136,14 @@
       aoff += wrap ? tap_step : 32 * ES;
       kc = wrap ? 0 : kc;
     };
-    auto step = [&](int d, int slot, bool more, bool reload, int knext) {
+    auto step = [&](int d, int slot, bool more, bool reload, int wv, int wc) {
       if (more) request((slot + PF) % NB);
       __builtin_amdgcn_sched_barrier(0);
 #pragma unroll
       for (int i = 0; i < NT; ++i)
 #pragma unroll
         for (int j = 0; j < MT; ++j) mma32(acc[i][j], q[d][i], a[slot][j]);
-      if (reload) load_chunk(d, knext);
+      if (reload) load_chunk(d, wv, wc);
       __builtin_amdgcn_sched_barrier(0);
     };
 #pragma unroll
@@ -133,10 +153,10 @@
 #pragma unroll 1
     for (int g = 0; g < G; ++g, kt += D) {
 #pragma unroll
-      for (int d = 0; d < D; ++d) step(d, d % NB, true, true, kt + d + D);
-    }
-#pragma unroll
-    for (int j = 0; j < KT_ - G * D; ++j) step(j % D, (G * D + j) % NB, G * D + j + PF < KT_, G * D + j + D < KT_, G * D + j + D);
+      for (int d = 0; d < D; ++d) step(d, d % NB, true, true, kt, d + D);
+    }
+#pragma unroll
+    for (int j = 0; j < KT_ - G * D; ++j) step(j % D, (G * D + j) % NB, G * D + j + PF < KT_, G * D + j + D < KT_, 0, G * D + j + D);
   }
   template <int MT, int KT_, int ABL = DHW_ABL>
   DHW_DEV void run_s(f32x4 (&acc)[NT][MT], const char* abase, int stride, int KC) {
@@ -150,7 +170,7 @@
     constexpr int G = NR / D;
     int aoff = 0, kc = 0;
     const int tap_step = stride - (KC - 1) * 32 * ES;
-    auto step = [&](int d, bool reload, int knext) {
+    auto step = [&](int d, bool reload, int wv, int wc) {
       Frag<T> a[MT];
 #pragma unroll
       for (int j = 0; j < MT; ++j) {
@@ -165,7 +185,7 @@
           else mma32(acc[i][j], q[d][i], a[j]);
         }
       if constexpr (!(ABL & 2)) {
-        if (reload) load_chunk(d, knext);
+        if (reload) load_chunk(d, wv, wc);
       }
       const bool wrap = ++kc == KC;
       aoff += wrap ? tap_step : 32 * ES;
@@ -175,16 +195,16 @@
 #pragma unroll 1
     for (int g = 0; g < G; ++g, kt += D) {
 #pragma unroll
-      for (int d = 0; d < D; ++d) step(d, true, kt + d + D);
-    }
-#pragma unroll
-    for (int j = 0; j < KT_ - G * D; ++j) step(j % D, G * D + j + D < KT_, G * D + j + D);
+      for (int d = 0; d < D; ++d) step(d, true, kt, d + D);
+    }
+#pragma unroll
+    for (int j = 0; j < KT_ - G * D; ++j) step(j % D, G * D + j + D < KT_, 0, G * D + j + D);
   }
 
   template <int KT_> static constexpr int eff_depth() { return D < KT_ ? D : KT_; }
 
   template <int MT, int KT_, int KTN_>
-  DHW_DEV void run_n(f32x4 (&acc)[NT][MT], const char* abase, int stride, int KC, const T* __restrict__ nbase, int nkts = 0) {
+  DHW_DEV void run_n(f32x4 (&acc)[NT][MT], const char* abase, int stride, int KC, Src nsrc, int nkts = 0) {
     static_assert(KT_ <= D, "run_n: the stage must fit the ring");
     constexpr int ES = sizeof(T), DN = eff_depth<KTN_>();
     constexpr int XTRA = DN > KT_ ? DN - KT_ : 0, PER = (XTRA + KT_ - 1) / KT_;
@@ -202,7 +222,10 @@
     };
     auto next_chunk = [&](int c) {
 #pragma unroll
-      for (int i = 0; i < NT; ++i) q[c][i] = frag_load(nbase + ((size_t)i * nKTS + c) * 512);
+      for (int i = 0; i < NT; ++i) {
+        if constexpr (UB) q[c][i] = wfrag_of(nsrc.base, nsrc.lane, i, nKTS, 0, c);
+        else q[c][i] = wfrag_of(nsrc, 0, i, nKTS, 0, c);
+      }
     };
 #pragma unroll
     for (int c = 0; c < PF; ++c)
@@ -221,7 +244,7 @@
         if (KT_ + s * PER + e < DN) next_chunk(KT_ + s * PER + e);
       __builtin_amdgcn_sched_barrier(0);
     }
-    base = nbase; KT = KTN_; KTS = nKTS;
+    src(nsrc); KT = KTN_; KTS = nKTS;
   }
 };
 
@@ -241,6 +264,30 @@
   for (int id = tid; id < total; id += nthreads) {
     const int r = id / cpr, cc = id - r * cpr;
     *reinterpret_cast<uint4*>(gdst + (size_t)r * gs + cc * EPV) = *reinterpret_cast<const uint4*>(lds + r * S + cc * 16);
+  }
+}
+template <typename T, int C>
+DHW_DEV void tile_copy_out_rows(const char* lds, int S, T* gdst, int rows_valid, int tid, int nthreads) {
+  constexpr int RB = C * (int)sizeof(T), cpr = RB / 16;
+  char* const g = reinterpret_cast<char*>(gdst);
+  const int total = rows_valid * cpr;
+  for (int id = tid; id < total; id += nthreads)
+    *reinterpret_cast<uint4*>(g + (uint32_t)(id * 16)) = *reinterpret_cast<const uint4*>(lds + id * 16 + (id / cpr) * (S - RB));
+}
+template <typename T, int C>
+DHW_DEV void tile_copy_out_pool_rows(const char* lds, int S, T* gdst, int rows_valid_in, int tid, int nthreads) {
+  constexpr int RB = C * (int)sizeof(T), cpr = RB / 16, EPV = 16 / (int)sizeof(T);
+  char* const g = reinterpret_cast<char*>(gdst);
+  const int total = (rows_valid_in / 2) * cpr;
+  for (int id = tid; id < total; id += nthreads) {
+    const char* src = lds + id * 16 + (id / cpr) * (2 * S - RB);
+    uint4 a = *reinterpret_cast<const uint4*>(src);
+    const uint4 b = *reinterpret_cast<const uint4*>(src + S);
+    T* ea = reinterpret_cast<T*>(&a);
+    const T* eb = reinterpret_cast<const T*>(&b);
+#pragma unroll
+    for (int k = 0; k < EPV; ++k) ea[k] = from_f<T>(0.5f * (to_f(ea[k]) + to_f(eb[k])));
+    *reinterpret_cast<uint4*>(g + (uint32_t)(id * 16)) = a;
   }
 }
 template <typename T>
```

Result: no change. 1.778 million stroke-points/s (-0.3%).
